# alexandervakhitov/lld-slam

Hardware: AMD Instinct MI355X
Metric: local-BA windows/sec (50 KF, 10k pts, 2k lines) at matched chi2; 1/2/4/8 GPU (higher is better)
Workload: dtype f64

## Files before the change

### lld_slam_amd/csrc/lld_ba.hip

```cpp
#include <algorithm>
#include <atomic>
#include <cfloat>
#include <chrono>
#include <cmath>
#include <cstdio>
#include <cstdlib>
#include <cstring>
#include <memory>
#include <mutex>
#include <new>
#include <thread>

#include "lld_ba_kernels.h"

using namespace lldba;

namespace {
constexpr int kNumPhases = 5;
constexpr int kFusePairsBelowWindows = 24;
constexpr int kMaxSuperSteps = 512;
constexpr int kChunkSmall = 4, kChunkFromWindows = 24;
constexpr int kSchurWindowTile = 8;
#ifdef LLD_EXPERIMENTS
static int exp_int(const char* name, int dflt) { const char* e = std::getenv(name); return e ? std::atoi(e) : dflt; }
// ... 431 lines not shown
    }
  if (!cholplan::build(n_free, adj, force, S.plan)) std::memset(&S.plan, 0, sizeof S.plan);
}

}


static void ba_drop_groups(lld_ba_batch* B) {
  for (auto& G : B->groups) {
    if (G.own_stream && G.st) (void)hipStreamSynchronize(G.st);
    if (G.gexec) { (void)hipGraphExecDestroy(G.gexec); G.gexec = nullptr; }
    if (G.graph) { (void)hipGraphDestroy(G.graph); G.graph = nullptr; }
    if (B->borrowed) continue;
    for (auto& row : G.ev) for (auto& e : row) if (e) (void)hipEventDestroy(e);
    if (G.own_stream && G.st) (void)hipStreamDestroy(G.st);
  }
  B->groups.clear();
}

static int ba_make_groups(lld_ba_batch* B, int n_groups) {
  const int n_windows = B->n_windows;
  int G = n_groups;
  if (G <= 0) {
    G = n_windows >= 16 ? 4 : (n_windows >= 8 ? 3 : 1);
    if (B->pipelined) G = std::min(G, 2);
    static const int groups_exp = exp_int("LLD_BA_GROUPS", 0);
    if (groups_exp >= 1 && groups_exp <= 8) G = groups_exp;
  }
  G = std::max(1, std::min(std::min(G, 8), n_windows));
  ba_drop_groups(B);
  B->groups.resize(G);
  for (int g = 0; g < G; g++) {
    lld_ba_batch::Group& Gr = B->groups[g];
    Gr.w0 = (int)((long long)n_windows * g / G); Gr.nw = (int)((long long)n_windows * (g + 1) / G) - Gr.w0;
    lld_ctx::BACache& cache = B->ctx->ba;
    if (g == 0) Gr.st = B->ctx->stream;
    else if (B->borrowed) {
      if (!cache.streams[g - 1]) LLD_HIP_TRY(hipStreamCreateWithFlags(&cache.streams[g - 1], hipStreamNonBlocking));
      Gr.st = cache.streams[g - 1]; Gr.own_stream = true;
    } else { LLD_HIP_TRY(hipStreamCreateWithFlags(&Gr.st, hipStreamNonBlocking)); Gr.own_stream = true; }
    Gr.d_counters = B->d_counters + 4 * g; Gr.h_counters = B->h_counters + 4 * g;
    static const int chunk_from = exp_int("LLD_BA_CHUNK_FROM", kChunkFromWindows);
    Gr.chunk0 = (B->pcg_multi || Gr.nw >= chunk_from) ? 1 : kChunkSmall; Gr.chunk = Gr.chunk0;
    Gr.chunk_from = chunk_from;
    for (int q = 0; q < Gr.chunk; q++)
      for (int k = 0; k < kNumPhases + 1; k++) {
        if (B->borrowed) { if (!cache.events[g][q][k]) LLD_HIP_TRY(hipEventCreate(&cache.events[g][q][k])); Gr.ev[q][k] = cache.events[g][q][k]; }
        else LLD_HIP_TRY(hipEventCreate(&Gr.ev[q][k]));
      }
    for (int wi = Gr.w0; wi < Gr.w0 + Gr.nw; wi++) {
      const BAWin& W = B->h_wins[wi];
      Gr.max_lblocks = std::max(Gr.max_lblocks, W.nb_pt + W.nb_ln);
      Gr.max_nt_pt = std::max(Gr.max_nt_pt, W.nt_pt); Gr.max_nb_ln = std::max(Gr.max_nb_ln, W.nt_ln);
      Gr.max_nl_pt = std::max(Gr.max_nl_pt, W.nl_pt); Gr.max_nl_ln = std::max(Gr.max_nl_ln, W.nl_ln);
      Gr.max_items_pt = std::max(Gr.max_items_pt, W.n_items_pt); Gr.max_items_ln = std::max(Gr.max_items_ln, W.n_items - W.n_items_pt);
      Gr.max_blk = std::max(Gr.max_blk, B->A.s_skip_empty ? W.n_blk_nz : W.n_free * (W.n_free + 1) / 2);
      const bool sp = (size_t)wi < B->plan_mode.size() && B->plan_mode[wi] == 1;
      Gr.any_sparse = Gr.any_sparse || sp; Gr.any_dense = Gr.any_dense || !sp;
    }
  }
  return LLD_OK;
}

extern "C" {

constexpr int kNotPacked = -1000;
static int ba_batch_create_impl(lld_ctx* ctx, int n_windows, const lld_ba_window* wins, const lld_ba_params* params, bool packed, lld_ba_batch** out) {
  if (!ctx || n_windows <= 0 || !wins || !out) return LLD_ERR_INVALID;
  *out = nullptr;
  for (int w = 0; w < n_windows; w++) { int st = validate_window(wins[w], false); if (st) return st; }
  LLD_HIP_TRY(hipSetDevice(ctx->device));
  static const bool timing = exp_flag("LLD_BA_TIMING");
  const auto tc0 = std::chrono::steady_clock::now();
  auto lap = [&](const char* what) { if (timing) std::fprintf(stderr, "[ba_create] %s at %.3f ms\n", what, std::chrono::duration<double, std::milli>(std::chrono::steady_clock::now() - tc0).count()); };
  lld_ba_batch* B = new lld_ba_batch();
  B->ctx = ctx; B->n_windows = n_windows;
  if (params) B->params = *params; else lld_ba_params_default(&B->params);
  const lld_ba_params& P = B->params;
  if (P.its_round1 < 1 || (P.protocol == 0 && P.its_round2 < 1) || P.its_round2 < 0 || P.max_trials <= 0 || !(P.pcg_rel_tol > 0) || P.reduced_solver < 0 || P.reduced_solver > 5 || P.protocol < 0 || P.protocol > 1 || P.abort_after_trials < 0) { delete B; return LLD_ERR_INVALID; }

  B->h_wins.resize(n_windows);
  B->chunk_landmarks = n_windows >= 64 ? 256 : (n_windows >= 8 ? 64 : 32);
  { static const int chunk_exp = exp_int("LLD_BA_CHUNK", 0); if (chunk_exp >= 1 && chunk_exp <= 4096) B->chunk_landmarks = chunk_exp; }
  std::vector<WinBases> bases(n_windows + 1);
  {
    WinBases b{};
    for (int wi = 0; wi < n_windows; wi++) {
      bases[wi] = b;
      const lld_ba_window& w = wins[wi];
      b.NC += w.n_cams; b.NP += w.n_points; b.NL += w.n_lines; b.NPE += w.n_pt_obs; b.NLO += w.n_ln_obs; b.NF += w.n_free_cams;
      const size_t n = 6 * (size_t)w.n_free_cams;
      b.S_total += n * n; b.x_total += n;
    }
    bases[n_windows] = b;
  }
  const long long NC = bases[n_windows].NC, NP = bases[n_windows].NP, NL = bases[n_windows].NL, NPE = bases[n_windows].NPE, NLO = bases[n_windows].NLO, NF = bases[n_windows].NF;
  if (NPE > 0x3fffffffll || NLO > 0x1fffffffll || NC * 7 > 0x7fffffffll) { delete B; return LLD_ERR_UNSUPPORTED; }
  const size_t S_total = bases[n_windows].S_total, x_total = bases[n_windows].x_total;
  const size_t NLE = 2 * (size_t)NLO;
  lld_ctx::BACache& cache = ctx->ba;
  const bool cached = !cache.busy.exchange(true);
  void* priv_stage[2] = {nullptr, nullptr};
  bool uploads_queued = false;
  auto fail = [&](int st) {
    if (uploads_queued) {
      (void)hipStreamSynchronize(ctx->stream);
      if (B->borrowed) cache.stage_pending = false;
    }
    for (void* q : priv_stage) if (q) (void)hipHostFree(q);
    ba_drop_groups(B);
    if (B->borrowed) cache.busy = false;
    else {
      if (B->h_counters) (void)hipHostFree(B->h_counters);
      if (B->slab) (void)hipFree(B->slab);
    }
    delete B; return st;
  };
  if (cached) B->borrowed = true;
  SecA hA{}, dA{};
  lld_slab dryA; dryA.base = reinterpret_cast<char*>(256);
  carve_a(dryA, packed, NC, NP, NL, NPE, NLE, hA);
  const size_t bytesA = dryA.used;
  void* arenaA = nullptr;
  { const int gs = stage_arena(ctx, cached, 0, bytesA, &arenaA); if (gs) return fail(gs); if (!cached) priv_stage[0] = arenaA; }
  { lld_slab sl; sl.base = static_cast<char*>(arenaA); sl.size = bytesA; carve_a(sl, packed, NC, NP, NL, NPE, NLE, hA); }
  HostArrays H;
  H.packed = packed;
  H.cam_qt0.view(hA.cam_qt0, 7 * (size_t)NC); H.pt0.view(hA.pt0, 3 * (size_t)NP); H.ln_x0.view(hA.ln_x0, 3 * (size_t)NL); H.ln_dir.view(hA.ln_dir, 3 * (size_t)NL);
  H.ln_info.view(hA.ln_info, 256);
  H.pt_obs_start.view(hA.pt_obs_start, (size_t)NP + 1); H.ln_obs_start.view(hA.ln_obs_start, (size_t)NL + 1);
  H.pe_pt.view(hA.pe_pt, NPE);
  if (packed) {
    H.pe_obs.view(hA.pe_obs, NPE); H.pe_cs.view(hA.pe_cs, NPE); H.lo_seg.view(hA.lo_seg, NLE); H.lo_cs.view(hA.lo_cs, NLO); H.lo_ln.view(hA.lo_ln, NLO); H.lo_oct.view(hA.lo_oct, NLO);
  } else {
    H.pe_cam.view(hA.pe_cam, NPE); H.pe_u.view(hA.pe_u, NPE); H.pe_v.view(hA.pe_v, NPE); H.pe_ur.view(hA.pe_ur, NPE); H.pe_s.view(hA.pe_s, NPE);
    H.le_cam.view(hA.le_cam, NLE); H.le_ln.view(hA.le_ln, NLE); H.le_xs.view(hA.le_xs, NLE); H.le_ys.view(hA.le_ys, NLE); H.le_xe.view(hA.le_xe, NLE); H.le_ye.view(hA.le_ye, NLE);
    H.le_s.view(hA.le_s, NLE);
  }
  H.pt_obs_start.p[NP] = (int)NPE; H.ln_obs_start.p[NL] = (int)NLO;
  for (int i = 0; i < 255; i++) H.ln_info.p[i] = P.protocol == 1 ? 1.0 : lld::line_info(P.gamma, i);
  H.ln_info.p[255] = 0.0;
  bool big_map = false;
  for (int wi = 0; wi < n_windows; wi++) {
    const size_t nf = (size_t)wins[wi].n_free_cams, nc = (size_t)wins[wi].n_cams;
    if (nf > (size_t)kMaxFreeCamsLds || (nf * 27 + 8 + nc * 7) * sizeof(double) > 158 * 1024 || (8 + nc * 14 + nf * 6) * sizeof(double) > 158 * 1024) big_map = true;
    B->max_free = std::max(B->max_free, wins[wi].n_free_cams); B->max_cams = std::max(B->max_cams, wins[wi].n_cams);
  }
  const bool force_big = exp_flag("LLD_BA_FORCE_BIG");
  if (force_big) big_map = true;
  B->big = big_map;
  if (P.deterministic < 0 || P.deterministic > 2) return fail(LLD_ERR_INVALID);
  if (B->big && P.deterministic == 1) return fail(LLD_ERR_UNSUPPORTED);
  const bool det = P.deterministic != 0 && !B->big;
  auto lin_lds_bytes = [&](int copies) { return ((size_t)B->max_free * 27 * copies + 8 + (size_t)B->max_cams * 7) * sizeof(double); };
  int copies = B->big ? 1 : kAccCopies;
  while (!B->big && copies > 1 && lin_lds_bytes(copies) > 150 * 1024) copies >>= 1;
  if (!B->big && lin_lds_bytes(copies) > 158 * 1024) return fail(LLD_ERR_UNSUPPORTED);
  B->acc_copies[0] = B->acc_copies[1] = copies;
  B->lin_waves[0] = det ? copies : kLinThreads / 64;
  B->lin_waves[1] = det ? copies : (n_windows >= 64 ? 4 : kLinThreads / 64);
  if (const char* e = exp_str("LLD_BA_LIN_WAVES")) {
    int a = 0, c = 0;
    if (std::sscanf(e, "%d,%d", &a, &c) == 2 && a >= 1 && a <= 8 && c >= 1 && c <= 8) {
      B->lin_waves[0] = a; B->lin_waves[1] = c;
      if (det) { B->acc_copies[0] = a; B->acc_copies[1] = c; if (lin_lds_bytes(std::max(a, c)) > 158 * 1024) return fail(LLD_ERR_UNSUPPORTED); }
    }
  }
  std::vector<WinStage> stages(n_windows);
  int n_threads = 1;
  const bool staged_under_solve = g_big_solves_running[ctx->device & 63].load(std::memory_order_relaxed) > 0;
  if (n_windows >= 4) {
    n_threads = (int)std::min<unsigned>(std::max(1u, std::thread::hardware_concurrency()), 16u);
    if (g_big_solves_running[ctx->device & 63].load(std::memory_order_relaxed) > 0) n_threads = std::min(n_threads, staging_cap());
    if (const char* e = std::getenv("LLD_HOST_THREADS")) { const int v = std::atoi(e); if (v >= 1 && v <= 64) n_threads = v; }
    if (g_big_solves_running[ctx->device & 63].load(std::memory_order_relaxed) > 0) n_threads = std::min(n_threads, staging_cap());
    n_threads = std::min(n_threads, n_windows);
  }
  std::atomic<int> first_error{LLD_OK};
  auto for_windows = [&](auto&& body) {
    std::atomic<int> next{0};
    auto worker = [&]() {
      for (;;) {
        const int wi = next.fetch_add(1);
        if (wi >= n_windows || first_error.load() != LLD_OK) break;
        try { body(wi); } catch (...) { int ok = LLD_OK; first_error.compare_exchange_strong(ok, LLD_ERR_ALLOC); }
      }
    };
    std::vector<std::thread> pool;
    try { for (int t = 1; t < n_threads; t++) pool.emplace_back(worker); } catch (...) {}
    worker();
    for (auto& t : pool) t.join();
  };
  void* const early_slab = (cached && n_windows >= 32 && cache.slab && cache.slab_bytes >= bytesA + 4096 && !exp_flag("LLD_BA_POISON") && !exp_flag("LLD_BA_NO_EARLY_UPLOAD")) ? cache.slab : nullptr;
  const int n_ranges = early_slab ? std::min(8, n_windows / 16) : 0;
  std::unique_ptr<std::atomic<int>[]> range_left(n_ranges ? new std::atomic<int>[(size_t)n_ranges] : nullptr);
  auto range_lo = [&](int r) { return (int)((long long)n_windows * r / std::max(1, n_ranges)); };
  for (int r = 0; r < n_ranges; r++) range_left[(size_t)r].store(range_lo(r + 1) - range_lo(r));
  auto copy_rows = [&](const void* hbase, size_t elt, long long lo, long long hi) -> bool {
    if (!hbase || hi <= lo) return true;
    const char* h = static_cast<const char*>(hbase) + elt * (size_t)lo;
    char* d = static_cast<char*>(early_slab) + (h - static_cast<const char*>(arenaA));
    return hipMemcpyAsync(d, h, elt * (size_t)(hi - lo), hipMemcpyHostToDevice, ctx->stream) == hipSuccess;
  };
  auto early_copy = [&](int r) {
    if (hipSetDevice(ctx->device) != hipSuccess) { int ok = LLD_OK; first_error.compare_exchange_strong(ok, LLD_ERR_HIP); return; }
    const WinBases& a = bases[(size_t)range_lo(r)]; const WinBases& b = bases[(size_t)range_lo(r + 1)];
    bool ok = copy_rows(hA.cam_qt0, 7 * sizeof(double), a.NC, b.NC) && copy_rows(hA.pt0, 3 * sizeof(double), a.NP, b.NP) &&
              copy_rows(hA.ln_x0, 3 * sizeof(double), a.NL, b.NL) && copy_rows(hA.ln_dir, 3 * sizeof(double), a.NL, b.NL) &&
              copy_rows(hA.pt_obs_start, sizeof(int), a.NP, b.NP) && copy_rows(hA.ln_obs_start, sizeof(int), a.NL, b.NL) && copy_rows(hA.pe_pt, sizeof(int), a.NPE, b.NPE);
    if (packed)
      ok = ok && copy_rows(hA.pe_obs, sizeof(float4), a.NPE, b.NPE) && copy_rows(hA.pe_cs, sizeof(int), a.NPE, b.NPE) && copy_rows(hA.lo_seg, sizeof(float4), 2 * a.NLO, 2 * b.NLO) &&
           copy_rows(hA.lo_cs, sizeof(int), a.NLO, b.NLO) && copy_rows(hA.lo_ln, sizeof(int), a.NLO, b.NLO) && copy_rows(hA.lo_oct, sizeof(unsigned short), a.NLO, b.NLO);
    else
      ok = ok && copy_rows(hA.pe_cam, sizeof(int), a.NPE, b.NPE) && copy_rows(hA.pe_u, sizeof(double), a.NPE, b.NPE) && copy_rows(hA.pe_v, sizeof(double), a.NPE, b.NPE) &&
           copy_rows(hA.pe_ur, sizeof(double), a.NPE, b.NPE) && copy_rows(hA.pe_s, sizeof(double), a.NPE, b.NPE) &&
           copy_rows(hA.le_cam, sizeof(int), 2 * a.NLO, 2 * b.NLO) && copy_rows(hA.le_ln, sizeof(int), 2 * a.NLO, 2 * b.NLO) &&
           copy_rows(hA.le_xs, sizeof(double), 2 * a.NLO, 2 * b.NLO) && copy_rows(hA.le_ys, sizeof(double), 2 * a.NLO, 2 * b.NLO) && copy_rows(hA.le_xe, sizeof(double), 2 * a.NLO, 2 * b.NLO) &&
           copy_rows(hA.le_ye, sizeof(double), 2 * a.NLO, 2 * b.NLO) && copy_rows(hA.le_s, sizeof(double), 2 * a.NLO, 2 * b.NLO);
    if (!ok) { int e_ = LLD_OK; first_error.compare_exchange_strong(e_, LLD_ERR_HIP); }
  };
  auto window_staged = [&](int wi) {
    if (!n_ranges) return;
    int r = (int)(((long long)wi * n_ranges) / n_windows);
    while (r + 1 < n_ranges && wi >= range_lo(r + 1)) r++;
    while (r > 0 && wi < range_lo(r)) r--;
    if (range_left[(size_t)r].fetch_sub(1) == 1) early_copy(r);
  };
  if (n_ranges) uploads_queued = true;
  const auto lap1 = [&](const char* what) { if (n_windows == 1) lap(what); };
  for_windows([&](int wi) {
    const int st = validate_window(wins[wi]);
    if (st) { int ok = LLD_OK; first_error.compare_exchange_strong(ok, st); return; }
    BAWin& W = B->h_wins[wi];
    WinStage& S = stages[wi];
    stage_tasks(wins[wi], P, bases[wi], n_windows, B->lin_waves, det, W, S);
    lap1("tasks built");
    if (n_windows == 1 && wins[wi].n_pt_obs + wins[wi].n_ln_obs > 20000) {
      std::thread helper;
      bool helped = false;
      try { helper = std::thread([&]() { try { stage_chunks(wins[wi], 3, bases[wi], B->chunk_landmarks, S.cs[0]); } catch (...) { int ok = LLD_OK; first_error.compare_exchange_strong(ok, LLD_ERR_ALLOC); } }); helped = true; } catch (...) {}
      if (!stage_edges(wins[wi], P, bases[wi], W, S, H)) { int ok = LLD_OK; first_error.compare_exchange_strong(ok, kNotPacked); }
      lap1("edges flattened");
      stage_chunks(wins[wi], 4, bases[wi], B->chunk_landmarks, S.cs[1]);
      if (helped) helper.join(); else stage_chunks(wins[wi], 3, bases[wi], B->chunk_landmarks, S.cs[0]);
    } else {
      if (!stage_edges(wins[wi], P, bases[wi], W, S, H)) { int ok = LLD_OK; first_error.compare_exchange_strong(ok, kNotPacked); return; }
      lap1("edges flattened");
      window_staged(wi);
      stage_chunks(wins[wi], 3, bases[wi], B->chunk_landmarks, S.cs[0]);
      stage_chunks(wins[wi], 4, bases[wi], B->chunk_landmarks, S.cs[1]);
    }
    stage_csr(wins[wi].n_free_cams, S);
    W.n_blk_nz = S.n_blk_nz;
    {
      static const int plan_force = exp_int("LLD_BA_CHOL_FORCE", 0);
      stage_chol_plan(wins[wi].n_free_cams, P.reduced_solver == 0 ? plan_force : (P.reduced_solver == 4 ? 1 : (P.reduced_solver == 5 ? 2 : 3)), S);
    }
    lap1("chunks built");
  });
  if (first_error.load() != LLD_OK) return fail(first_error.load());
  struct Place { size_t ptask, ltask, chunk, lm, tab, cams, blk_start, blk_src, cam_start, cam_src, part, cpart; };
  std::vector<Place> place(n_windows + 1);
  size_t n_hpart = 0; long long NPART = 0; int max_blk = 0;
  {
    Place q{};
    for (int wi = 0; wi < n_windows; wi++) {
      place[wi] = q;
      const WinStage& S = stages[wi];
      BAWin& W = B->h_wins[wi];
      W.ptask_off = (int)q.ptask; W.ltask_off = (int)q.ltask; W.item_off = (int)q.chunk;
      W.n_items_pt = (int)S.cs[0].chunks.size(); W.n_items = W.n_items_pt + (int)S.cs[1].chunks.size();
      W.blk_csr_off = (int)q.blk_start; W.cam_csr_off = (int)q.cam_start;
      W.hpart_off = (long long)n_hpart; n_hpart += (size_t)(big_map ? 1 : W.nl_pt + W.nl_ln) * W.n_free * 27;
      W.part_off = (int)NPART; NPART += W.nt_pt + W.nt_ln;
      q.ptask += S.ptasks.size(); q.ltask += S.ltasks.size(); q.chunk += (size_t)W.n_items;
      q.lm += S.cs[0].sg_lm.size() + S.cs[1].sg_lm.size(); q.tab += S.cs[0].sg_tab.size() + S.cs[1].sg_tab.size(); q.cams += S.cs[0].sg_cams.size() + S.cs[1].sg_cams.size();
      q.blk_start += S.blk_start.size(); q.blk_src += S.blk_src.size(); q.cam_start += S.cam_start.size(); q.cam_src += S.cam_src.size();
      q.part += S.cs[0].n_part + S.cs[1].n_part; q.cpart += S.cs[0].n_cpart + S.cs[1].n_cpart;
      if (q.part * 4 > 0x7fffffffull || q.tab > 0x7fffffffull) return fail(LLD_ERR_UNSUPPORTED);
      for (int d = 0; d < 2; d++) B->schur_lds[d] = std::max(B->schur_lds[d], S.cs[d].lds_need);
      for (int d = 0; d < 2; d++) B->schur_wide_lds = std::max(B->schur_wide_lds, S.cs[d].wide_lds_need);
      if (B->schur_wide_lds > 64 * 1024) return fail(LLD_ERR_UNSUPPORTED);
      max_blk = std::max(max_blk, W.n_free * (W.n_free + 1) / 2);
      B->max_items_pt = std::max(B->max_items_pt, W.n_items_pt); B->max_items_ln = std::max(B->max_items_ln, W.n_items - W.n_items_pt);
      B->max_lblocks = std::max(B->max_lblocks, W.nb_pt + W.nb_ln);
      B->max_free = std::max(B->max_free, W.n_free);
      B->max_cams = std::max(B->max_cams, W.n_cams);
      B->rec_stride = std::max(B->rec_stride, record_bytes(W));
    }
    place[n_windows] = q;
  }
  const Place& tot = place[n_windows];
  const size_t n_part = tot.part, n_cpart = tot.cpart;
  B->pcg_multi = n_windows <= 8 && B->max_free * 6 > kCholMN && P.reduced_solver != 2;
  const bool s_skip_empty = (P.reduced_solver == 0 || P.reduced_solver >= 3) && B->max_free * 6 <= kCholMN && !B->pcg_multi;
  if (B->max_free > kMaxFreeCamsOneWg && !B->pcg_multi) return fail(LLD_ERR_UNSUPPORTED);
  if (B->max_cams > kPcgThreads && !B->pcg_multi) return fail(LLD_ERR_UNSUPPORTED);
  for (int wi = 0; wi < n_windows; wi++) { B->h_wins[wi].acc_copies[0] = B->acc_copies[0]; B->h_wins[wi].acc_copies[1] = B->acc_copies[1]; B->h_wins[wi].win_index = wi; B->h_wins[wi].big = B->big ? 1 : 0; }
  B->max_blk = max_blk;
  for (int wi = 0; wi < n_windows; wi++) B->h_wins[wi].rec_off = (long long)(B->rec_stride * (size_t)wi);
  const size_t rec_total = B->rec_stride * (size_t)n_windows;
  B->S_total = S_total; B->x_total = x_total;
  const SecBSizes zB{tot.blk_start, tot.blk_src, tot.cam_start, tot.cam_src, tot.lm, tot.tab, tot.cams, tot.chunk, tot.ptask, tot.ltask, n_windows};
  hipStream_t st = ctx->stream;
  BAArrays& A = B->A;
  SecB dB{};
  size_t offA = 0, offB = 0, bytesB = 0;
  auto carve = [&](lld_slab& sl) {
    std::memset(&A, 0, sizeof A);
    offA = sl.used; carve_a(sl, packed, NC, NP, NL, NPE, NLE, dA);
    offB = sl.used; carve_b(sl, zB, dB); bytesB = sl.used - offB;
    A.cam_qt0 = dA.cam_qt0; A.pt0 = dA.pt0; A.ln_x0 = dA.ln_x0; A.ln_dir = dA.ln_dir; A.pt_obs_start = dA.pt_obs_start; A.ln_obs_start = dA.ln_obs_start;
    A.pe_pt = dA.pe_pt; A.ln_info = dA.ln_info; A.packed = packed ? 1 : 0;
    A.pe_obs = dA.pe_obs; A.pe_cs = dA.pe_cs; A.lo_seg = dA.lo_seg; A.lo_cs = dA.lo_cs; A.lo_ln = dA.lo_ln; A.lo_oct = dA.lo_oct;
    A.pe_cam = dA.pe_cam; A.pe_u = dA.pe_u; A.pe_v = dA.pe_v; A.pe_ur = dA.pe_ur; A.pe_s = dA.pe_s;
    A.le_cam = dA.le_cam; A.le_ln = dA.le_ln; A.le_xs = dA.le_xs; A.le_ys = dA.le_ys; A.le_xe = dA.le_xe; A.le_ye = dA.le_ye; A.le_s = dA.le_s;
    A.blk_start = dB.blk_start; A.blk_perm = dB.blk_perm; A.blk_src = dB.blk_src; A.cam_start = dB.cam_start; A.cam_src = dB.cam_src;
    A.sg_lm = dB.sg_lm; A.sg_tab = dB.sg_tab; A.sg_cams = dB.sg_cams; A.sg_chunks = dB.chunks; A.ptasks = dB.ptasks; A.ltasks = dB.ltasks;
    B->d_wins = dB.wins; A.chol_plan = dB.plans;
    B->d_state = sl.take<BAState>(n_windows);
    A.NC = NC; A.NP = NP; A.NL = NL;
    A.cam_qt = sl.take<double>(2 * NC * 7 + 1);
    A.ptx = sl.take<double>(2 * NP + 1); A.pty = sl.take<double>(2 * NP + 1); A.ptz = sl.take<double>(2 * NP + 1);
    A.lqx = sl.take<double>(2 * NL + 1); A.lqy = sl.take<double>(2 * NL + 1); A.lqz = sl.take<double>(2 * NL + 1); A.lqw = sl.take<double>(2 * NL + 1); A.lal = sl.take<double>(2 * NL + 1);
    A.pe_flags = sl.take<uint8_t>(NPE + 1); A.le_flags = sl.take<uint8_t>(NLE + 1);
    A.pe_chi2 = sl.take<double>(NPE + 1); A.le_chi2 = sl.take<double>(NLE + 1);
    A.pe_ws = sl.take<double>((size_t)NPE + 1); A.lo_W = sl.take<double>((size_t)NLO * 24 + 1);
    A.pt_active = sl.take<uint8_t>(NP + 1); A.ln_active = sl.take<uint8_t>(NL + 1); A.ln_removed = sl.take<uint8_t>(NL + 1);
    A.pt_V = sl.take<double>((size_t)NP * 9 + 1); A.ln_V = sl.take<double>((size_t)NL * 14 + 1);
    A.hpp_part = sl.take<double>(n_hpart + 2);
    A.Hpp = sl.take<double>((size_t)NF * 21 + 1); A.bp = sl.take<double>((size_t)NF * 6 + 1);
    A.S = sl.take<double>(S_total + 1); A.bschur = sl.take<double>(x_total + 1); A.xp = sl.take<double>(x_total + 1);
    A.x_total = (long long)x_total; A.s_skip_empty = s_skip_empty ? 1 : 0;
    if (B->pcg_multi) { A.pcg_vec = sl.take<double>(4 * x_total + 4); A.pcg_mi = sl.take<double>((size_t)NF * 36 + 1); A.pcg_sc = sl.take<double>(8 * (size_t)n_windows + 8); }
    A.chi_part = sl.take<double>(NPART + 1); A.chi_part2 = sl.take<double>(NPART + 1); A.scale_part = sl.take<double>(NPART + 1);
    A.sp_part = sl.take<double>(n_part * 36 + 2); A.sp_cpart = sl.take<double>(n_cpart * 6 + 2);
    A.records = sl.take<unsigned char>(rec_total + 256);
#ifdef LLD_EXPERIMENTS
    A.chol_stamps = exp_flag("LLD_BA_CHOL_STAMPS") ? sl.take<long long>((size_t)n_windows * kCholStampWaves * kCholStampSlots) : nullptr;
#endif
    B->d_counters = sl.take<int>(4 * 8);
    B->d_slot_map = sl.take<int>(2 * ((size_t)n_windows + 1)); B->d_active_pub = sl.take<int>((size_t)n_windows + 1);
  };
  lap("host staging done");
  lld_slab dry; dry.base = reinterpret_cast<char*>(256);
  carve(dry);
  const size_t bytes = dry.used + 4096;
  bool slab_regrown = false;
  if (cached) {
    if (bytes > cache.slab_bytes) {
      slab_regrown = true;
      void* old_slab = cache.slab;
      cache.slab = nullptr; cache.slab_bytes = 0;
      if (old_slab && hipFree(old_slab) != hipSuccess) return fail(LLD_ERR_HIP);
      const size_t want = bytes + (bytes >> 4);
      if (hipMalloc(&cache.slab, want) != hipSuccess) return fail(LLD_ERR_ALLOC);
      cache.slab_bytes = want;
    }
    B->slab = cache.slab;
  } else if (hipMalloc(&B->slab, bytes) != hipSuccess) return fail(LLD_ERR_ALLOC);
  B->slab_bytes = bytes;
  lap("slab ready");
  const bool poison = exp_flag("LLD_BA_POISON");
  if (poison && hipMemsetAsync(B->slab, 0xFF, bytes, st) != hipSuccess) return fail(LLD_ERR_HIP);
  lld_slab sl; sl.base = (char*)B->slab; sl.size = bytes;
  carve(sl);
#ifdef LLD_EXPERIMENTS
  if (A.chol_stamps && hipMemsetAsync(A.chol_stamps, 0, sizeof(long long) * (size_t)n_windows * kCholStampWaves * kCholStampSlots, st) != hipSuccess) return fail(LLD_ERR_HIP);
#endif
  if (s_skip_empty && S_total > 0 && hipMemsetAsync(A.S, 0, S_total * sizeof(double), st) != hipSuccess) return fail(LLD_ERR_HIP);
  uploads_queued = true;
  if (n_ranges && !slab_regrown && B->slab == early_slab && offA == 0) {
    bool ok = copy_rows(hA.ln_info, sizeof(double), 0, 256) && copy_rows(hA.pt_obs_start, sizeof(int), NP, NP + 1) && copy_rows(hA.ln_obs_start, sizeof(int), NL, NL + 1);
    if (!ok) return fail(LLD_ERR_HIP);
  } else if (hipMemcpyAsync((char*)B->slab + offA, arenaA, bytesA, hipMemcpyHostToDevice, st) != hipSuccess) return fail(LLD_ERR_HIP);
  lap("inputs queued");
  void* arenaB = nullptr;
  { const int gs = stage_arena(ctx, cached, 1, bytesB, &arenaB); if (gs) return fail(gs); if (!cached) priv_stage[1] = arenaB; }
  SecB hB{};
  B->plan_mode.assign((size_t)n_windows, 0);
  { lld_slab slb; slb.base = static_cast<char*>(arenaB); slb.size = bytesB; carve_b(slb, zB, hB); }
  hB.blk_start[tot.blk_start] = (int)tot.blk_src; hB.cam_start[tot.cam_start] = (int)tot.cam_src;
  for_windows([&](int wi) {
    const Place& q = place[wi];
    WinStage& S = stages[wi];
    std::copy(S.ptasks.begin(), S.ptasks.end(), hB.ptasks + q.ptask);
    std::copy(S.ltasks.begin(), S.ltasks.end(), hB.ltasks + q.ltask);
    size_t at_chunk = q.chunk, at_lm = q.lm, at_tab = q.tab, at_cams = q.cams;
    for (int d = 0; d < 2; d++) {
      const ChunkStage& C = S.cs[d];
      for (SChunk c : C.chunks) {
        c.lm_off += (int)at_lm; c.tab_off += (int)at_tab; c.cams_off += (int)at_cams; c.part_off += (int)q.part; c.cpart_off += (int)q.cpart;
        hB.chunks[at_chunk++] = c;
      }
      std::copy(C.sg_lm.begin(), C.sg_lm.end(), hB.sg_lm + at_lm); at_lm += C.sg_lm.size();
      std::copy(C.sg_tab.begin(), C.sg_tab.end(), hB.sg_tab + at_tab); at_tab += C.sg_tab.size();
      std::copy(C.sg_cams.begin(), C.sg_cams.end(), hB.sg_cams + at_cams); at_cams += C.sg_cams.size();
    }
    const int part4 = (int)(q.part * 4), cpart0 = (int)q.cpart, bsrc0 = (int)q.blk_src, csrc0 = (int)q.cam_src;
    for (size_t i = 0; i < S.blk_start.size(); i++) hB.blk_start[q.blk_start + i] = S.blk_start[i] + bsrc0;
    for (size_t i = 0; i < S.blk_perm.size(); i++) hB.blk_perm[q.blk_start + i] = S.blk_perm[i];
    for (size_t i = 0; i < S.blk_src.size(); i++) hB.blk_src[q.blk_src + i] = S.blk_src[i] + part4;
    for (size_t i = 0; i < S.cam_start.size(); i++) hB.cam_start[q.cam_start + i] = S.cam_start[i] + csrc0;
    for (size_t i = 0; i < S.cam_src.size(); i++) hB.cam_src[q.cam_src + i] = S.cam_src[i] + cpart0;
    hB.wins[wi] = B->h_wins[wi];
    hB.plans[wi] = S.plan; B->plan_mode[wi] = S.plan.mode;
    S = WinStage();
  });
  if (first_error.load() != LLD_OK) return fail(first_error.load());
  stages.clear();
  if (hipMemcpyAsync((char*)B->slab + offB, arenaB, bytesB, hipMemcpyHostToDevice, st) != hipSuccess) return fail(LLD_ERR_HIP);
  lap("structures queued");
  if (!cache.attrs_set || !cached) {
    const int lds_max = 159 * 1024;
    const void* fns[] = {reinterpret_cast<const void*>(ba_pcg_kernel), reinterpret_cast<const void*>(ba_backsub_pt_kernel), reinterpret_cast<const void*>(ba_backsub_ln_kernel),
                         reinterpret_cast<const void*>(ba_backsub_ctl_kernel), reinterpret_cast<const void*>(ba_linearize_pt_kernel), reinterpret_cast<const void*>(ba_linearize_ln_kernel),
                         reinterpret_cast<const void*>(ba_linearize_both_kernel), reinterpret_cast<const void*>(ba_backsub_pt_f64_kernel), reinterpret_cast<const void*>(ba_backsub_ln_f64_kernel),
                         reinterpret_cast<const void*>(ba_linearize_pt_f64_kernel), reinterpret_cast<const void*>(ba_linearize_ln_f64_kernel), reinterpret_cast<const void*>(ba_chol_kernel), reinterpret_cast<const void*>(ba_chol_mfma_kernel), reinterpret_cast<const void*>(ba_chol_sparse_kernel),
    };
    for (const void* f : fns) if (hipFuncSetAttribute(f, hipFuncAttributeMaxDynamicSharedMemorySize, lds_max) != hipSuccess) return fail(LLD_ERR_HIP);
    if (cached) cache.attrs_set = true;
  }
  lap("attributes set");
  if (B->borrowed) {
    if (!ctx->poll && hipHostMalloc(&ctx->poll, 256, hipHostMallocDefault) != hipSuccess) return fail(LLD_ERR_HIP);
    B->h_counters = static_cast<int*>(ctx->poll);
  } else if (hipHostMalloc((void**)&B->h_counters, 256, hipHostMallocDefault) != hipSuccess) return fail(LLD_ERR_HIP);
  B->h_abort = B->h_counters + 48;
  lap("pinned counters");
  B->pipelined = n_windows >= kSerialiseSolvesFromWindows && (staged_under_solve || g_big_solves_running[ctx->device & 63].load(std::memory_order_relaxed) > 0);
  { int gs = ba_make_groups(B, 0); if (gs) return fail(gs); }
  lap("groups made");
  if (cached) {
    if (!cache.stage_free && hipEventCreateWithFlags(&cache.stage_free, hipEventDisableTiming) != hipSuccess) return fail(LLD_ERR_HIP);
    if (hipEventRecord(cache.stage_free, st) != hipSuccess) return fail(LLD_ERR_HIP);
    cache.stage_pending = true;
  } else {
    if (hipStreamSynchronize(st) != hipSuccess) return fail(LLD_ERR_HIP);
    for (void*& q : priv_stage) if (q) { (void)hipHostFree(q); q = nullptr; }
  }
  lap("done");
  *out = B;
  return LLD_OK;
}

static int ba_batch_create_any(lld_ctx* ctx, int n_windows, const lld_ba_window* wins, const lld_ba_params* params, lld_ba_batch** out) {
  const bool f64_only = exp_flag("LLD_BA_OBS_F64");
  int st = f64_only ? kNotPacked : ba_batch_create_impl(ctx, n_windows, wins, params, true, out);
  if (st == kNotPacked) st = ba_batch_create_impl(ctx, n_windows, wins, params, false, out);
  return st;
}

int lld_ba_batch_create(lld_ctx* ctx, int n_windows, const lld_ba_window* wins, const lld_ba_params* params, lld_ba_batch** out) {
  return ba_batch_create_any(ctx, n_windows, wins, params, out);
}

struct StopFlag {
  volatile const int* i32; volatile const unsigned char* u8;
  bool up() const { return (i32 && *i32) || (u8 && *u8); }
};

static int ba_batch_solve_body(lld_ba_batch* B, StopFlag abort_flag, hipEvent_t t_begin, hipEvent_t t_end) {
  lld_ctx* ctx = B->ctx;
  std::unique_lock<std::mutex> turn(g_big_solve[ctx->device & 63], std::defer_lock);
  struct RunningGuard { std::atomic<int>* c; ~RunningGuard() { if (c) c->fetch_sub(1, std::memory_order_relaxed); } } running{nullptr};
  if (B->n_windows >= kSerialiseSolvesFromWindows) {
    turn.lock();
    running.c = &g_big_solves_running[ctx->device & 63]; running.c->fetch_add(1, std::memory_order_relaxed);
  }
  BAArrays& A = B->A;
  B->records_valid = false;
  for (auto& m : B->phase_ms) m = 0.0;
  for (auto& l : B->launches) l = 0;
  B->super_steps = 0;
  LLD_HIP_TRY(hipEventRecord(t_begin, ctx->stream));
  const size_t lin_lds_pt = B->big ? 64 : ((size_t)B->max_free * 27 * B->acc_copies[0] + 8 + (size_t)B->max_cams * 7) * sizeof(double);
  const size_t lin_lds_ln = B->big ? 64 : ((size_t)B->max_free * 27 * B->acc_copies[1] + 8 + (size_t)B->max_cams * 7) * sizeof(double);
  const bool same_lin_shape = B->lin_waves[0] == B->lin_waves[1] && B->acc_copies[0] == B->acc_copies[1];
  const size_t bs_lds = B->big ? 64 : (8 + (size_t)B->max_cams * 14 + (size_t)B->max_free * 6) * sizeof(double);
  const size_t pcg_lds = ((size_t)B->max_free * 6 * 4 + kPcgThreads + (size_t)B->max_free * 36 + 32) * sizeof(double);
  const size_t chol_fixed = ((size_t)B->max_free * 36 * 2 + (size_t)B->max_free * 6 * 2 + 32) * sizeof(double);
  const size_t chol_tri = std::min((size_t)B->max_free * (B->max_free + 1) / 2 * 36 * sizeof(double), (size_t)(156 * 1024) - chol_fixed) / 288 * 288;
  const size_t chol_lds = chol_fixed + chol_tri;
  const bool abort_at_start = abort_flag.up();
  *B->h_abort = 0;
  const bool live_flag = abort_flag.i32 != nullptr || abort_flag.u8 != nullptr;
  using Group = lld_ba_batch::Group;

  auto finalize_group = [&](Group& G) {
    const BAWin* dw = B->d_wins + G.w0; BAState* ds = B->d_state + G.w0;
    hipLaunchKernelGGL(ba_finalize_kernel, dim3(G.max_lblocks + 1, G.nw), dim3(kLmThreads), 0, G.st, A, dw, ds);
    hipLaunchKernelGGL(ba_mark_done_kernel, dim3((G.nw + 63) / 64), dim3(64), 0, G.st, ds, G.nw);
  };
  const bool use_slots = !(B->params.reduced_solver == 1 || B->pcg_multi);
  auto group_arrays = [&](const Group& G) { BAArrays Ag = B->A; int* rd = B->d_slot_map + (size_t)G.map_parity * ((size_t)B->n_windows + 1) + G.w0;
                                            int* wr = B->d_slot_map + (size_t)(G.map_parity ^ 1) * ((size_t)B->n_windows + 1) + G.w0;
                                            Ag.slot_map = use_slots ? wr : nullptr; Ag.active_pub = use_slots ? B->d_active_pub + G.w0 : nullptr;
                                            Ag.slot_rd = (use_slots && G.rows < G.nw) ? rd : nullptr; return Ag; };
  static const bool use_graph = exp_flag("LLD_BA_GRAPH");
  bool capturing = false;
  int n_superstep_launches = 0;
  const int fail_at = exp_int("LLD_BA_FAIL_AT_SUPERSTEP", -1);
  auto launch_superstep = [&](Group& G, int q) -> int {
    const BAWin* dw = B->d_wins + G.w0; BAState* ds = B->d_state + G.w0;
    if (fail_at >= 0 && n_superstep_launches++ == fail_at) return LLD_ERR_UNSUPPORTED;
    const BAArrays A = group_arrays(G);
    const int nw = use_slots ? std::max(1, std::min(G.rows, G.nw)) : G.nw; hipStream_t st = G.st;
    const int abort_now = abort_flag.up() ? 1 : 0;
    hipEvent_t* ev = G.ev[q];
    const bool tev = B->phase_events && !capturing;
    if (tev) LLD_HIP_TRY(hipEventRecord(ev[0], st));
    static const int fuse_below = exp_int("LLD_BA_FUSE_BELOW", kFusePairsBelowWindows);
    const bool packed = A.packed != 0;
    const bool fuse_pairs = nw < fuse_below && !B->big && packed;
    static const int fuse_bs_below = exp_int("LLD_BA_FUSE_BS_BELOW", -1);
    const bool fuse_bs = fuse_bs_below >= 0 ? (nw < fuse_bs_below && !B->big && packed) : fuse_pairs;
    if (B->big) {
      if (G.max_nl_pt > 0) hipLaunchKernelGGL(ba_linearize_pt_big_kernel, dim3(G.max_nl_pt, nw), dim3(64 * B->lin_waves[0]), lin_lds_pt, st, A, dw, ds);
      if (G.max_nl_ln > 0) hipLaunchKernelGGL(ba_linearize_ln_big_kernel, dim3(G.max_nl_ln, nw), dim3(64 * B->lin_waves[1]), lin_lds_ln, st, A, dw, ds);
    } else if (fuse_pairs && same_lin_shape && G.max_nl_pt > 0 && G.max_nl_ln > 0) hipLaunchKernelGGL(ba_linearize_both_kernel, dim3(G.max_nl_pt + G.max_nl_ln, nw), dim3(64 * B->lin_waves[0]), lin_lds_pt, st, A, dw, ds, G.max_nl_pt);
    else {
      if (G.max_nl_pt > 0) hipLaunchKernelGGL(packed ? ba_linearize_pt_kernel : ba_linearize_pt_f64_kernel, dim3(G.max_nl_pt, nw), dim3(64 * B->lin_waves[0]), lin_lds_pt, st, A, dw, ds);
      if (G.max_nl_ln > 0) hipLaunchKernelGGL(packed ? ba_linearize_ln_kernel : ba_linearize_ln_f64_kernel, dim3(G.max_nl_ln, nw), dim3(64 * B->lin_waves[1]), lin_lds_ln, st, A, dw, ds);
    }
    hipLaunchKernelGGL(ba_hpp_reduce_kernel, dim3(std::max(1, (B->max_free * 27 + 255) / 256), nw), dim3(256), 0, st, A, dw, ds);
    if (tev) LLD_HIP_TRY(hipEventRecord(ev[1], st));
    static const int schur_tile = std::max(1, exp_int("LLD_BA_SCHUR_TILE", kSchurWindowTile));
    static const bool split_schur = exp_flag("LLD_BA_SPLIT_SCHUR");
    if (split_schur) {
      if (G.max_items_pt > 0) hipLaunchKernelGGL(ba_schur_items_kernel<3>, dim3(G.max_items_pt, nw), dim3(kSchurThreads), B->schur_lds[0], st, A, dw, ds);
      if (G.max_items_ln > 0) hipLaunchKernelGGL(ba_schur_items_kernel<4>, dim3(G.max_items_ln, nw), dim3(kSchurThreads), B->schur_lds[1], st, A, dw, ds);
    } else if (G.max_items_pt + G.max_items_ln > 0) {
      if ((long long)nw * (G.max_items_pt + G.max_items_ln) * kSchurThreads > 0xffffffffll) return LLD_ERR_UNSUPPORTED;
      hipLaunchKernelGGL(ba_schur_items_both_kernel, dim3((unsigned)((long long)nw * (G.max_items_pt + G.max_items_ln))), dim3(kSchurThreads), std::max(B->schur_lds[0], B->schur_lds[1]), st, A, dw, ds, G.max_items_pt, schur_tile, nw, G.max_items_pt + G.max_items_ln);
    }
    if (B->schur_wide_lds > 0) hipLaunchKernelGGL(ba_schur_wide_kernel, dim3(G.max_items_pt + G.max_items_ln, nw), dim3(kSchurWideThreads), B->schur_wide_lds, st, A, dw, ds);
    hipLaunchKernelGGL(ba_schur_reduce_kernel, dim3((std::max(1, G.max_blk) * 6 + 255) / 256 + 2, nw), dim3(256), 0, st, A, dw, ds);
    if (B->params.reduced_solver == 1 || B->pcg_multi) hipLaunchKernelGGL(ba_symmetrize_kernel, dim3(B->pcg_multi ? 256 : 16, nw), dim3(256), 0, st, A, dw, ds);
    if (tev) LLD_HIP_TRY(hipEventRecord(ev[2], st));
    if (B->pcg_multi) {
      hipLaunchKernelGGL(ba_pcgm_init_kernel, dim3(nw), dim3(kPcgThreads), 0, st, A, dw, ds, B->params.pcg_rel_tol);
      const int n_max = B->max_free * 6, limit = B->params.pcg_max_iter > 0 ? B->params.pcg_max_iter : 10 * n_max;
      std::vector<double> hsc(8 * (size_t)nw);
      for (int it = 0; it < limit;) {
        for (int k = 0; k < 16 && it < limit; k++, it++) {
          hipLaunchKernelGGL(ba_pcgm_matvec_kernel, dim3((n_max + 3) / 4, nw), dim3(256), 0, st, A, dw);
          hipLaunchKernelGGL(ba_pcgm_update_kernel, dim3(nw), dim3(kPcgThreads), 0, st, A, dw, B->params.pcg_max_iter);
        }
        LLD_HIP_TRY(hipMemcpyAsync(hsc.data(), A.pcg_sc + 8 * (size_t)G.w0, hsc.size() * sizeof(double), hipMemcpyDeviceToHost, st));
        LLD_HIP_TRY(hipStreamSynchronize(st));
        bool all_done = true;
        for (int wI = 0; wI < nw; wI++) all_done = all_done && hsc[8 * (size_t)wI + 3] != 0.0;
        if (all_done) break;
      }
      hipLaunchKernelGGL(ba_pcgm_final_kernel, dim3(nw), dim3(kPcgThreads), 0, st, A, dw, ds);
    } else if (B->params.reduced_solver == 1)
      hipLaunchKernelGGL(ba_pcg_kernel, dim3(nw), dim3(kPcgThreads), pcg_lds, st, A, dw, ds, B->params.pcg_rel_tol, B->params.pcg_max_iter);
    else if ((B->params.reduced_solver == 0 || B->params.reduced_solver >= 3) && B->max_free * 6 <= kCholMN) {
      if (G.any_sparse) hipLaunchKernelGGL(ba_chol_sparse_kernel, dim3(nw), dim3(kSpThreads), kSpLdsBytes, st, A, dw, ds);
      if (G.any_dense) hipLaunchKernelGGL(ba_chol_mfma_kernel, dim3(nw), dim3(kCholMThreads), kCholMLdsDoubles * sizeof(double), st, A, dw, ds);
    }
    else
      hipLaunchKernelGGL(ba_chol_kernel, dim3(nw), dim3(kPcgThreads), chol_lds, st, A, dw, ds, (int)(chol_tri / sizeof(double)));
    if (tev) LLD_HIP_TRY(hipEventRecord(ev[3], st));
    bool control_fused = false;
    if (B->big) {
      if (G.max_nt_pt > 0) hipLaunchKernelGGL(ba_backsub_pt_big_kernel, dim3(G.max_nt_pt, nw), dim3(kLmThreads), bs_lds, st, A, dw, ds);
      if (G.max_nb_ln > 0) hipLaunchKernelGGL(ba_backsub_ln_big_kernel, dim3(G.max_nb_ln, nw), dim3(kLmThreads), bs_lds, st, A, dw, ds);
    } else if (fuse_bs && G.max_nt_pt > 0 && G.max_nb_ln > 0) {
      hipLaunchKernelGGL(ba_backsub_ctl_kernel, dim3(G.max_nt_pt + G.max_nb_ln, nw), dim3(kLmThreads), bs_lds, st, A, dw, ds, G.max_nt_pt, abort_now, G.nw, G.d_counters, G.h_counters,
                         (live_flag && G.chunk > 1) ? B->h_abort : nullptr);
      control_fused = true;
    }
    else {
      if (G.max_nt_pt > 0) hipLaunchKernelGGL(packed ? ba_backsub_pt_kernel : ba_backsub_pt_f64_kernel, dim3(G.max_nt_pt, nw), dim3(kLmThreads), bs_lds, st, A, dw, ds);
      if (G.max_nb_ln > 0) hipLaunchKernelGGL(packed ? ba_backsub_ln_kernel : ba_backsub_ln_f64_kernel, dim3(G.max_nb_ln, nw), dim3(kLmThreads), bs_lds, st, A, dw, ds);
    }
    if (tev) LLD_HIP_TRY(hipEventRecord(ev[4], st));
    if (!control_fused)
      hipLaunchKernelGGL(ba_control_kernel, dim3(nw), dim3(kCtlThreads), 0, st, A, dw, ds, abort_now, G.nw, G.d_counters, G.h_counters, (live_flag && G.chunk > 1) ? B->h_abort : nullptr);
    if (G.chunk > 1) {
      hipLaunchKernelGGL(ba_classify_kernel, dim3(std::max(1, G.max_lblocks), nw), dim3(kLmThreads), 0, st, A, dw, ds);
    }
    LLD_HIP_TRY(hipGetLastError());
    if (!capturing && (tev || q == G.chunk - 1)) LLD_HIP_TRY(hipEventRecord(ev[5], st));
    G.map_parity ^= 1;
    return LLD_OK;
  };
  auto launch_chunk = [&](Group& G) -> int {
    if (use_graph && G.chunk > 1 && (G.chunk & 1) == 0) {
      if (!G.gexec) {
        G.rows = G.nw;
        LLD_HIP_TRY(hipStreamBeginCapture(G.st, hipStreamCaptureModeThreadLocal));
        capturing = true;
        int s_ = LLD_OK;
        for (int q = 0; q < G.chunk && s_ == LLD_OK; q++) s_ = launch_superstep(G, q);
        capturing = false;
        LLD_HIP_TRY(hipStreamEndCapture(G.st, &G.graph));
        if (s_) return s_;
        LLD_HIP_TRY(hipGraphInstantiate(&G.gexec, G.graph, nullptr, nullptr, 0));
      }
      LLD_HIP_TRY(hipGraphLaunch(G.gexec, G.st));
      LLD_HIP_TRY(hipEventRecord(G.ev[G.chunk - 1][5], G.st));
      return LLD_OK;
    }
    for (int q = 0; q < G.chunk; q++) { const int s_ = launch_superstep(G, q); if (s_) return s_; }
    return LLD_OK;
  };

  for (Group& G : B->groups) {
    const BAWin* dw = B->d_wins + G.w0; BAState* ds = B->d_state + G.w0;
    if (G.own_stream) LLD_HIP_TRY(hipStreamWaitEvent(G.st, t_begin, 0));
    G.steps = 0; G.active = !abort_at_start; G.rows = G.nw; G.chunk = G.chunk0; G.map_parity = 0;
    LLD_HIP_TRY(hipMemsetAsync(G.d_counters, 0, 4 * sizeof(int), G.st));
    hipLaunchKernelGGL(ba_init_kernel, dim3(std::max(1, std::min(64, G.max_lblocks + 1)), G.nw), dim3(kLmThreads), 0, G.st, group_arrays(G), dw, ds);
    LLD_HIP_TRY(hipGetLastError());
    if (abort_at_start) {
      std::vector<BAState> hs(G.nw);
      std::memset(hs.data(), 0, sizeof(BAState) * G.nw);
      for (auto& s : hs) { s.phase = PH_FINALIZE; s.aborted = 1; }
      LLD_HIP_TRY(hipMemcpyAsync(ds, hs.data(), sizeof(BAState) * G.nw, hipMemcpyHostToDevice, G.st));
      LLD_HIP_TRY(hipStreamSynchronize(G.st));
      finalize_group(G);
    } else {
      int s = launch_chunk(G); if (s) return s;
    }
  }
  for (bool any = !abort_at_start; any;) {
    any = false;
    for (Group& G : B->groups) {
      if (!G.active) continue;
      if (live_flag && G.chunk > 1) {
        for (;;) {
          const hipError_t q = hipEventQuery(G.ev[G.chunk - 1][5]);
          if (q == hipSuccess) break;
          if (q != hipErrorNotReady) LLD_HIP_TRY(q);
          if (abort_flag.up()) __atomic_store_n(B->h_abort, 1, __ATOMIC_RELEASE);
          std::this_thread::yield();
        }
      } else LLD_HIP_TRY(hipEventSynchronize(G.ev[G.chunk - 1][5]));
      for (int q = 0; q < G.chunk; q++)
        for (int k = 0; k < kNumPhases; k++) {
          float ms = 0.f;
          if (B->phase_events && hipEventElapsedTime(&ms, G.ev[q][k], G.ev[q][k + 1]) == hipSuccess) B->phase_ms[k] += ms;
          B->launches[k]++;
        }
      G.steps += G.chunk; B->super_steps += G.chunk;
      const int n_run = G.h_counters[0], n_trans = G.h_counters[1], n_fin = G.h_counters[2];
      const BAWin* dw = B->d_wins + G.w0; BAState* ds = B->d_state + G.w0;
      if (use_slots && !(use_graph && G.gexec)) G.rows = n_run + n_trans;
      if (turn.owns_lock() && use_slots) {
        int left = 0;
        for (const Group& Gq : B->groups) left += Gq.active ? Gq.rows : 0;
        if (left * 8 <= B->n_windows) turn.unlock();
      }
      if (n_trans > 0 && G.chunk == 1) {
        hipLaunchKernelGGL(ba_classify_kernel, dim3(std::max(1, G.max_lblocks), use_slots ? std::max(1, G.rows) : G.nw), dim3(kLmThreads), 0, G.st, group_arrays(G), dw, ds);
      }
      (void)n_fin;
      LLD_HIP_TRY(hipGetLastError());
      if ((n_run + n_trans) > 0 && G.steps < kMaxSuperSteps) { int s = launch_chunk(G); if (s) return s; any = true; }
      else G.active = false;
    }
  }
  for (Group& G : B->groups) {
    finalize_group(G);
    LLD_HIP_TRY(hipGetLastError());
    if (G.own_stream) { LLD_HIP_TRY(hipEventRecord(G.ev[0][0], G.st)); LLD_HIP_TRY(hipStreamWaitEvent(ctx->stream, G.ev[0][0], 0)); }
  }
  LLD_HIP_TRY(hipEventRecord(t_end, ctx->stream));
  LLD_HIP_TRY(hipEventSynchronize(t_end));
  float tot = 0.f;
  (void)hipEventElapsedTime(&tot, t_begin, t_end);
// ... 238 lines not shown
```

### lld_slam_amd/csrc/lld_ba_kernels.h

```cpp
#ifndef LLD_BA_KERNELS_H
#define LLD_BA_KERNELS_H

#include "lld_common.h"
#include "lld_device_math.h"
#include "lld_ba_chol_plan.h"

namespace lldba {

using namespace lld;

constexpr int kLmThreads = 256;
constexpr int kSchurThreads = 64;
constexpr int kSchurWideThreads = 256;
constexpr int kPcgThreads = 1024;
constexpr int kCtlThreads = 64;
constexpr int kLinThreads = 512;
constexpr int kRoundsThroughput[4] = {8, 2, 4, 1};
constexpr int kRoundsLatency[4] = {4, 2, 4, 1};
constexpr int kRoundsThroughputMinWindows = 32;
constexpr int kRoundsThroughputBig[4] = {16, 4, 16, 1};
constexpr int kRoundsBigMinWindows = 192;
constexpr int kAccCopies = 4;
constexpr int kAccCopiesDoc = 4;
constexpr int kMaxFreeCams = 8192;
constexpr int kMaxFreeCamsLds = 590;
constexpr int kMaxFreeCamsOneWg = 170;

enum Phase : int { PH_RUN = 0, PH_TRANSITION = 2, PH_FINALIZE = 3, PH_DONE = 4 };
constexpr uint8_t EF_LEVEL1 = 1, EF_ROBUST = 2, EF_VALID = 4, EF_PAIRSTEREO = 8, EF_STEREO = 16;

struct BAWin {
  CamK cam;
  int n_cams, n_free;
  int cam_off;
  int pt_off, n_pt;
  int ln_off, n_ln;
  int pe_off, n_pe;
  int le_off, n_le;
  int hpp_off;
  int x_off;
  long long S_off;
  int item_off, n_items, n_items_pt;
  int lo_off, n_lo;
  int blk_csr_off, cam_csr_off;
  int n_blk_nz;
  int nb_pt, nb_ln;
  int ptask_off, n_ptasks, nt_pt;
  int ltask_off, n_ltasks, nt_ln;
  int nl_pt, nl_ln;
  int rounds[4];
  long long hpart_off;
  int part_off;
  int its[2];
  int max_trials, ln_filter;
  int abort_after;
  int big;
  int protocol, robust_pts;
  int acc_copies[2];
  int det, lin_waves[2];
  int win_index;
  double th_mono, th_stereo;
  double th_ln_mono, th_ln_stereo;
  long long rec_off;
};

struct BAState {
  int phase, need_lin, round, it, q, cur, nBad, pcg_ok;
  double lambda, ni, currentChi, iniChi, scale_cam;
  unsigned long long maxdiag_bits;
  double chi2_round1, chi2_final;
  int lm_iterations[2], lm_trials[2];
  int pcg_iterations, aborted, n_active_edges, pad;
  int ticket_lin, ticket_bs, ticket_cls, pad2;
};

struct PTask { int l0, nl, e0, ne, ms, pad0, pad1, pad2; };

struct SChunk { int lm_off, n_lm, tab_off, cams_off, k, D, part_off, cpart_off; };

struct BAArrays {
  long long NC, NP, NL;
  double* cam_qt;
  double *ptx, *pty, *ptz;
  double *lqx, *lqy, *lqz, *lqw, *lal;
  const double* cam_qt0;
  const double* pt0;
  const double *ln_x0, *ln_dir;
  const int* pt_obs_start;
  const int* ln_obs_start;
  const int* pe_pt;
  int packed;
  int* slot_map;
  int* active_pub;
  const int* slot_rd;
  const float4* pe_obs;
  const int* pe_cs;
  const float4* lo_seg;
  const int* lo_cs;
  const int* lo_ln;
  const unsigned short* lo_oct;
  const double* ln_info;
  const int* pe_cam;
  const double *pe_u, *pe_v, *pe_ur, *pe_s;
  const int* le_cam; const int* le_ln;
  const double *le_xs, *le_ys, *le_xe, *le_ye, *le_s;
  uint8_t *pe_flags, *le_flags;
  double *pe_chi2, *le_chi2;
  double *pe_ws;
  double *lo_W;
  uint8_t *pt_active, *ln_active, *ln_removed;
  double *pt_V;
  double *ln_V;
  double *hpp_part;
  double *Hpp;
  double *bp;
  double *S, *bschur, *xp;
  double *pcg_vec;
  double *pcg_mi;
  double *pcg_sc;
  long long x_total;
  double *chi_part, *chi_part2, *scale_part;
  const SChunk* sg_chunks;
  const PTask* ptasks; const PTask* ltasks;
  double *sp_part, *sp_cpart;
  const int *blk_start, *blk_src, *cam_start, *cam_src;
  int s_skip_empty;
  const int *blk_perm;
  const int *sg_lm, *sg_tab, *sg_cams;
  const CholPlan* chol_plan;
  unsigned char* records;
#ifdef LLD_EXPERIMENTS
  long long* chol_stamps;
#endif
};
constexpr int kCholStampSlots = 256;
constexpr int kCholStampWaves = 16;
#ifdef LLD_EXPERIMENTS
#define LLD_CHOL_STAMP(k) do { if (stamp_base && lane == 0) stamp_base[(k)] = (long long)__builtin_amdgcn_s_memtime(); } while (0)
#else
#define LLD_CHOL_STAMP(k) do { } while (0)
#endif

__device__ __forceinline__ void xwg_store(double* p, double v) { __hip_atomic_store(p, v, __ATOMIC_RELAXED, __HIP_MEMORY_SCOPE_AGENT); }
__device__ __forceinline__ double xwg_load(const double* p) { return __hip_atomic_load(p, __ATOMIC_RELAXED, __HIP_MEMORY_SCOPE_AGENT); }
__device__ __forceinline__ void xwg_stores_done() { asm volatile("s_waitcnt vmcnt(0)" ::: "memory"); }
__device__ __forceinline__ void xwg_store_i32(int* p, int v) { __hip_atomic_store(p, v, __ATOMIC_RELAXED, __HIP_MEMORY_SCOPE_AGENT); }
__device__ __forceinline__ int xwg_load_i32(const int* p) { return __hip_atomic_load(p, __ATOMIC_RELAXED, __HIP_MEMORY_SCOPE_AGENT); }
#define LLD_ROW_WINDOW(A, st, y) ((A).slot_rd ? (A).slot_rd[(y)] : (int)(y))
__device__ __forceinline__ double wave_sum(double x) {
#pragma unroll
  for (int off = 32; off > 0; off >>= 1) x += __shfl_xor(x, off);
  return x;
}
__device__ __forceinline__ double wave_max(double x) {
#pragma unroll
  for (int off = 32; off > 0; off >>= 1) x = fmax(x, __shfl_xor(x, off));
  return x;
}
__device__ __forceinline__ double block_sum(double x, double* scratch) {
  const int lane = threadIdx.x & 63, wave = threadIdx.x >> 6, nw = blockDim.x >> 6;
  x = wave_sum(x);
  __syncthreads();
  if (lane == 0) scratch[wave] = x;
  __syncthreads();
  double t = 0.0;
  for (int i = 0; i < nw; i++) t += scratch[i];
  return t;
}
__device__ __forceinline__ double block_max(double x, double* scratch) {
  const int lane = threadIdx.x & 63, wave = threadIdx.x >> 6, nw = blockDim.x >> 6;
  x = wave_max(x);
  __syncthreads();
  if (lane == 0) scratch[wave] = x;
  __syncthreads();
  double t = 0.0;
  for (int i = 0; i < nw; i++) t = fmax(t, scratch[i]);
  return t;
}

template <int D>
__device__ __forceinline__ bool spd_inverse(const double* A, double* Ainv) {
  double L[D][D];
  bool ok = true;
#pragma unroll
  for (int j = 0; j < D; j++) {
    double d = A[j * D + j];
#pragma unroll
    for (int k = 0; k < j; k++) d -= L[j][k] * L[j][k];
    if (!(d > 0.0)) ok = false;
    const double ljj = sqrt(d);
    L[j][j] = ljj;
    const double inv = 1.0 / ljj;
#pragma unroll
    for (int i = j + 1; i < D; i++) {
      double s = A[i * D + j];
#pragma unroll
      for (int k = 0; k < j; k++) s -= L[i][k] * L[j][k];
      L[i][j] = s * inv;
    }
  }
  double Li[D][D];
#pragma unroll
  for (int j = 0; j < D; j++) {
    Li[j][j] = 1.0 / L[j][j];
#pragma unroll
    for (int i = j + 1; i < D; i++) {
      double s = 0.0;
#pragma unroll
      for (int k = j; k < i; k++) s -= L[i][k] * Li[k][j];
      Li[i][j] = s / L[i][i];
    }
  }
#pragma unroll
  for (int i = 0; i < D; i++)
#pragma unroll
    for (int j = i; j < D; j++) {
      double s = 0.0;
#pragma unroll
      for (int k = j; k < D; k++) s += Li[k][i] * Li[k][j];
      Ainv[i * D + j] = s; Ainv[j * D + i] = s;
    }
  return ok;
}

template <int D>
__device__ __forceinline__ void chol_packed(const double* U, double lambda, double* L, double* idiag) {
  double F[D][D];
  int kk = 0;
#pragma unroll
  for (int i = 0; i < D; i++)
#pragma unroll
    for (int j = i; j < D; j++) { F[j][i] = U[kk++]; }
#pragma unroll
  for (int i = 0; i < D; i++) F[i][i] += lambda;
#pragma unroll
  for (int j = 0; j < D; j++) {
    double d = F[j][j];
#pragma unroll
    for (int m = 0; m < j; m++) d -= L[j * (j + 1) / 2 + m] * L[j * (j + 1) / 2 + m];
    const double inv = rsqrt_nr(d);
    idiag[j] = inv;
#pragma unroll
    for (int i = j + 1; i < D; i++) {
      double sacc = F[i][j];
#pragma unroll
      for (int m = 0; m < j; m++) sacc -= L[i * (i + 1) / 2 + m] * L[j * (j + 1) / 2 + m];
      L[i * (i + 1) / 2 + j] = sacc * inv;
    }
  }
}
template <int D>
__device__ __forceinline__ void chol_solve(const double* U, double lambda, const double* t, double* x) {
  double L[D * (D + 1) / 2], idg[D], y[D];
  chol_packed<D>(U, lambda, L, idg);
#pragma unroll
  for (int c = 0; c < D; c++) {
    double sacc = t[c];
#pragma unroll
    for (int m = 0; m < c; m++) sacc -= y[m] * L[c * (c + 1) / 2 + m];
    y[c] = sacc * idg[c];
  }
#pragma unroll
  for (int c = D - 1; c >= 0; c--) {
    double sacc = y[c];
#pragma unroll
    for (int m = c + 1; m < D; m++) sacc -= x[m] * L[m * (m + 1) / 2 + c];
    x[c] = sacc * idg[c];
// ... 128 lines not shown
```

### lld_slam_amd/csrc/lld_ba_lines.h

```cpp

struct LineGeom { Vec3 c0, c1, X1, X2; double alpha; };
__device__ __forceinline__ LineGeom line_geom(const LineQ& L) {
  const Mat3 Rl = line_rotation_t<true>(L);
  LineGeom G; G.c0 = mat_col(Rl, 0); G.c1 = mat_col(Rl, 1); G.alpha = L.alpha; G.X1 = L.alpha * G.c1; G.X2 = G.X1 + G.c0;
  return G;
}
struct LnObsIn { uint8_t fl[2]; double xs[2], ys[2], xe[2], ye[2], s[2]; };
template <int kPk>
__device__ __forceinline__ void line_obs_load(const BAArrays& A, int o, LnObsIn& I) {
#pragma unroll
  for (int side = 0; side < 2; side++) {
    const int e = 2 * o + side;
    I.fl[side] = A.le_flags[e];
    const LnSeg g = ln_seg_of<kPk>(A, e);
    I.xs[side] = g.xs; I.ys[side] = g.ys; I.xe[side] = g.xe; I.ye[side] = g.ye;
  }
  if (obs_packed<kPk>(A)) { const unsigned oc = A.lo_oct[o]; I.s[0] = A.ln_info[oc & 255u]; I.s[1] = A.ln_info[oc >> 8]; }
  else { I.s[0] = A.le_s[2 * o]; I.s[1] = A.le_s[2 * o + 1]; }
}
__device__ __forceinline__ double line_obs_linearize(const BAArrays& A, const BAWin& W, const Pose& T, int o, int c, const LineGeom& G, const LnObsIn& I,
                                                     double* hb, double* acc_lds) {
  const bool free_cam = c < W.n_free;
  double Wo[24], Jc0[12], r0[2] = {0.0, 0.0}, ws0 = 0.0;
#pragma unroll
  for (int i = 0; i < 24; i++) Wo[i] = 0.0;
#pragma unroll
  for (int i = 0; i < 12; i++) Jc0[i] = 0.0;
  double chi = 0.0;
  const Mat3 Rc = quat_rotation(T.q);
  const Vec3 X1m = pose_map(T, G.X1), X2m = pose_map(T, G.X2);
#pragma unroll
  for (int side = 0; side < 2; side++) {
    const int e = 2 * o + side;
    const uint8_t fl = I.fl[side];
    if (!(fl & EF_VALID) || (fl & EF_LEVEL1)) continue;
    double r[2]; LineAdj adj;
    line_residual_t<true>(W.cam, side == 1 ? W.cam.bx_right : 0.0, X1m, X2m, I.xs[side], I.ys[side], I.xe[side], I.ye[side], r, &adj);
    const double s = I.s[side];
    const double c2 = chi2_of(r, 2, s);
    A.le_chi2[e] = c2;
    double w = 1.0, rho0 = c2;
    if (fl & EF_ROBUST) rho0 = huber_nr(c2, (fl & EF_PAIRSTEREO) ? W.th_ln_stereo : W.th_ln_mono, &w);
    chi += rho0;
    const double ws = w * s;
    double Jc[12], Jl[8];
    line_jac_pose(adj, X1m, X2m, Jc);
    line_jac_line(adj, Rc, G.c0, G.c1, G.alpha, Jl);
    int k = 0;
#pragma unroll
    for (int a = 0; a < 4; a++) {
      hb[10 + a] -= ws * (Jl[a] * r[0] + Jl[4 + a] * r[1]);
#pragma unroll
      for (int d = a; d < 4; d++) hb[k++] += ws * (Jl[a] * Jl[d] + Jl[4 + a] * Jl[4 + d]);
    }
    if (free_cam) {
#pragma unroll
      for (int rr = 0; rr < 6; rr++)
#pragma unroll
        for (int a = 0; a < 4; a++) Wo[rr * 4 + a] += ws * (Jc[rr] * Jl[a] + Jc[6 + rr] * Jl[4 + a]);
      if (side == 0) {
#pragma unroll
        for (int i = 0; i < 12; i++) Jc0[i] = Jc[i];
        r0[0] = r[0]; r0[1] = r[1]; ws0 = ws;
      } else {
        double* ac = acc_lds + c * 27;
        int kk = 0;
#pragma unroll
        for (int rr = 0; rr < 6; rr++) {
          atomicAdd(&ac[21 + rr], -(ws0 * (Jc0[rr] * r0[0] + Jc0[6 + rr] * r0[1]) + ws * (Jc[rr] * r[0] + Jc[6 + rr] * r[1])));
#pragma unroll
          for (int cc = rr; cc < 6; cc++)
            atomicAdd(&ac[kk++], ws0 * (Jc0[rr] * Jc0[cc] + Jc0[6 + rr] * Jc0[6 + cc]) + ws * (Jc[rr] * Jc[cc] + Jc[6 + rr] * Jc[6 + cc]));
        }
        ws0 = 0.0;
      }
    }
  }
  if (free_cam) {
    double* Wb = A.lo_W + (size_t)o * 24;
#pragma unroll
    for (int i = 0; i < 24; i += 2) *reinterpret_cast<double2*>(Wb + i) = make_double2(Wo[i], Wo[i + 1]);
    if (ws0 != 0.0) {
      double* ac = acc_lds + c * 27;
      int kk = 0;
#pragma unroll
      for (int rr = 0; rr < 6; rr++) {
        atomicAdd(&ac[21 + rr], -ws0 * (Jc0[rr] * r0[0] + Jc0[6 + rr] * r0[1]));
#pragma unroll
        for (int cc = rr; cc < 6; cc++) atomicAdd(&ac[kk++], ws0 * (Jc0[rr] * Jc0[cc] + Jc0[6 + rr] * Jc0[6 + cc]));
      }
    }
  }
  return chi;
}

template <bool kBig, int kPk>
__device__ __forceinline__ void ba_linearize_ln_body(const BAArrays& A, const BAWin* __restrict__ wins, BAState* __restrict__ st, const int bx) {
  extern __shared__ __attribute__((aligned(16))) double lds[];
  const int wrow = LLD_ROW_WINDOW(A, st, blockIdx.y);
  if (wrow < 0) return;
  const BAWin W = wins[wrow];
  BAState& S = st[wrow];
  if (S.phase != PH_RUN || !S.need_lin) return;
  if ((int)bx >= W.nl_ln) return;
  const int nacc = W.n_free * 27;
  double* acc_all = kBig ? A.hpp_part + W.hpart_off : lds;
  const int copies = W.acc_copies[1];
  double* scratch = kBig ? lds : lds + copies * nacc;
  double* acc = acc_all;
  const int cur = S.cur;
  double* cams_l = scratch + 8;
  const double* cams = kBig ? A.cam_qt + ((size_t)cur * A.NC + W.cam_off) * 7 : cams_l;
  const int nthr = blockDim.x, nwv = W.lin_waves[1];
  if (!kBig) {
    for (int i = threadIdx.x; i < copies * nacc; i += nthr) acc_all[i] = 0.0;
    acc = acc_all + (W.det ? (int)(threadIdx.x >> 6) : (int)((threadIdx.x >> 3) & (copies - 1))) * nacc;
    for (int i = threadIdx.x; i < W.n_cams * 7; i += nthr) cams_l[i] = A.cam_qt[((size_t)cur * A.NC + W.cam_off) * 7 + i];
  }
  __syncthreads();
  const int lane = threadIdx.x & 63;
  double chi = 0.0, maxd = 0.0;
  for (int rnd = 0; rnd < W.rounds[1]; rnd++) {
    const int ti = (bx * W.rounds[1] + rnd) * nwv + __builtin_amdgcn_readfirstlane(threadIdx.x >> 6);
    if (ti >= W.n_ltasks) break;
    const PTask T = A.ltasks[W.ltask_off + ti];
    double hb[14];
#pragma unroll
    for (int i = 0; i < 14; i++) hb[i] = 0.0;
    if (T.nl > 1) {
      const bool has = lane < T.ne;
      const int o = T.e0 + (has ? lane : 0);
      int c, l_raw;
      ln_cam_lm_of<kPk>(A, o, T.l0, c, l_raw);
      LnObsIn I;
      line_obs_load<kPk>(A, o, I);
      const int l = has ? l_raw : -1 - lane;
      const int g = W.ln_off + (has ? l : T.l0);
      const LineQ Lq = load_ln(A, cur, g);
      const bool lm_act = has && A.ln_active[g];
      if (lm_act) chi += line_obs_linearize(A, W, pose_load(cams + c * 7), o, c, line_geom(Lq), I, hb, acc);
      seg_sum<14>(hb, l, lane, T.ms);
      if (lm_act && o == A.ln_obs_start[g]) {
        double* V = A.ln_V + (size_t)g * 14;
#pragma unroll
        for (int i = 0; i < 14; i++) V[i] = hb[i];
        maxd = fmax(maxd, fmax(fmax(fabs(hb[0]), fabs(hb[4])), fmax(fabs(hb[7]), fabs(hb[9]))));
      }
    } else {
      const int g = W.ln_off + T.l0;
      if (A.ln_active[g]) {
        const LineGeom G = line_geom(load_ln(A, cur, g));
        for (int sidx = lane; sidx < T.ne; sidx += 64) {
          const int o = T.e0 + sidx, c = ln_cam_of<kPk>(A, o);
          LnObsIn I;
          line_obs_load<kPk>(A, o, I);
          chi += line_obs_linearize(A, W, pose_load(cams + c * 7), o, c, G, I, hb, acc);
        }
        wave_sum_n<14>(hb);
        if (lane == 0) {
          double* V = A.ln_V + (size_t)g * 14;
#pragma unroll
          for (int i = 0; i < 14; i++) V[i] = hb[i];
          maxd = fmax(maxd, fmax(fmax(fabs(hb[0]), fabs(hb[4])), fmax(fabs(hb[7]), fabs(hb[9]))));
        }
      }
    }
  }
  const double chi_t = block_sum(chi, scratch);
  const double max_t = block_max(maxd, scratch);
  if (threadIdx.x == 0) {
    A.chi_part[W.part_off + W.nl_pt + bx] = chi_t;
    atomicMax(&S.maxdiag_bits, (unsigned long long)__double_as_longlong(max_t));
  }
  __syncthreads();
  if (kBig) return;
  double* dst = A.hpp_part + W.hpart_off + (size_t)(W.nl_pt + bx) * nacc;
  for (int i = threadIdx.x; i < nacc; i += nthr) {
    double v = 0.0;
    for (int q = 0; q < copies; q++) v += acc_all[q * nacc + i];
    dst[i] = v;
  }
}
__global__ __launch_bounds__(kLinThreads) void ba_linearize_ln_kernel(BAArrays A, const BAWin* __restrict__ wins, BAState* __restrict__ st) { ba_linearize_ln_body<false, 1>(A, wins, st, (int)blockIdx.x); }
__global__ __launch_bounds__(kLinThreads) void ba_linearize_ln_f64_kernel(BAArrays A, const BAWin* __restrict__ wins, BAState* __restrict__ st) { ba_linearize_ln_body<false, 0>(A, wins, st, (int)blockIdx.x); }
__global__ __launch_bounds__(kLinThreads) void ba_linearize_ln_big_kernel(BAArrays A, const BAWin* __restrict__ wins, BAState* __restrict__ st) { ba_linearize_ln_body<true, kPkRuntime>(A, wins, st, (int)blockIdx.x); }

__device__ __forceinline__ void line_obs_wtx(const BAArrays& A, const BAWin& W, int o, int c, const double* xp, double* t) {
  const double* Wb = A.lo_W + (size_t)o * 24;
#pragma unroll
  for (int k = 0; k < 4; k++) {
    double s = 0.0;
#pragma unroll
    for (int r = 0; r < 6; r++) s += Wb[r * 4 + k] * xp[c * 6 + r];
    t[k] = s;
  }
}
__device__ __forceinline__ double line_obs_trial(const BAArrays& A, const BAWin& W, const Pose& T, int o, const LineGeom& G, const LnObsIn& I) {
  double chi = 0.0;
  const Vec3 X1m = pose_map(T, G.X1), X2m = pose_map(T, G.X2);
#pragma unroll
  for (int side = 0; side < 2; side++) {
    const int e = 2 * o + side;
    const uint8_t fl = I.fl[side];
    if (!(fl & EF_VALID) || (fl & EF_LEVEL1)) continue;
    double r[2];
    line_residual_t<true>(W.cam, side == 1 ? W.cam.bx_right : 0.0, X1m, X2m, I.xs[side], I.ys[side], I.xe[side], I.ye[side], r, nullptr);
    const double c2 = chi2_of(r, 2, I.s[side]);
    A.le_chi2[e] = c2;
    double w, rho0 = c2;
    if (fl & EF_ROBUST) rho0 = huber_nr(c2, (fl & EF_PAIRSTEREO) ? W.th_ln_stereo : W.th_ln_mono, &w);
    chi += rho0;
  }
  return chi;
}
__device__ __forceinline__ double line_backsub(const double* V, double lambda, const double* wtx, const LineQ& L, LineQ& Ln) {
  double t[4], xl[4], sc = 0.0;
#pragma unroll
  for (int i = 0; i < 4; i++) t[i] = V[10 + i] - wtx[i];
  chol_solve<4>(V, lambda, t, xl);
#pragma unroll
  for (int i = 0; i < 4; i++) sc += xl[i] * (lambda * xl[i] + V[10 + i]);
  Ln = line_oplus(L, xl);
  return sc;
}

template <bool kBig, int kPk>
__device__ __forceinline__ void ba_backsub_ln_body(const BAArrays& A, const BAWin* __restrict__ wins, const BAState* __restrict__ st, const int bx) {
  extern __shared__ __attribute__((aligned(16))) double lds[];
  double* scratch = lds;
  const int wrow = LLD_ROW_WINDOW(A, st, blockIdx.y);
  if (wrow < 0) return;
  const BAWin W = wins[wrow];
  const BAState& S = st[wrow];
  if (S.phase != PH_RUN) return;
  if ((int)bx >= W.nt_ln) return;
  const int cur = S.cur, nxt = cur ^ 1;
  const double lambda = S.lambda;
  double* camB_l = lds + 8; double* xps_l = camB_l + W.n_cams * 7;
  const double* camB = kBig ? A.cam_qt + ((size_t)nxt * A.NC + W.cam_off) * 7 : camB_l;
  const double* xp = kBig ? A.xp + W.x_off : xps_l;
  const int task_wave = __builtin_amdgcn_readfirstlane(threadIdx.x >> 6);
  PTask T_next = A.ltasks[W.ltask_off + min((bx * W.rounds[3]) * 4 + task_wave, W.n_ltasks - 1)];
  if (!kBig) {
    for (int i = threadIdx.x; i < W.n_cams * 7; i += kLmThreads) camB_l[i] = A.cam_qt[((size_t)nxt * A.NC + W.cam_off) * 7 + i];
    for (int i = threadIdx.x; i < 6 * W.n_free; i += kLmThreads) xps_l[i] = A.xp[W.x_off + i];
  }
  __syncthreads();
  const int lane = threadIdx.x & 63;
  double chi = 0.0, sc = 0.0;
  for (int rnd = 0; rnd < W.rounds[3]; rnd++) {
    const int ti = (bx * W.rounds[3] + rnd) * 4 + task_wave;
    if (ti >= W.n_ltasks) break;
    const PTask T = T_next;
    T_next = A.ltasks[W.ltask_off + min((bx * W.rounds[3] + rnd + 1) * 4 + task_wave, W.n_ltasks - 1)];
    if (T.nl > 1) {
      const bool has = lane < T.ne;
      const int o = T.e0 + (has ? lane : 0);
      int c, l_raw;
      ln_cam_lm_of<kPk>(A, o, T.l0, c, l_raw);
      LnObsIn I;
      line_obs_load<kPk>(A, o, I);
      const bool lmk = lane < T.nl;
      const int g2 = W.ln_off + T.l0 + (lmk ? lane : 0);
      const LineQ L2 = load_ln(A, cur, g2);
      const int act2 = lmk ? (int)A.ln_active[g2] : 0;
      const int start2 = A.ln_obs_start[g2], end2 = A.ln_obs_start[g2 + 1];
      const int l = has ? l_raw : -1 - lane;
      const int slot = has ? l - T.l0 : 0;
      const bool lm_act = has && __shfl(act2, slot) != 0;
      double wtx[4] = {0, 0, 0, 0};
      if (lm_act && c < W.n_free) line_obs_wtx(A, W, o, c, xp, wtx);
      double V2[14];
#pragma unroll
      for (int i = 0; i < 14; i++) V2[i] = A.ln_V[(size_t)g2 * 14 + i];
      seg_sum<4>(wtx, l, lane, T.ms);
      const int first = (lmk && end2 > start2) ? start2 - T.e0 : 0;
      double wl[4];
#pragma unroll
      for (int i = 0; i < 4; i++) wl[i] = __shfl(wtx[i], first);
      LineQ Ln2 = L2;
      if (lmk) {
        if (act2 && end2 > start2) sc += line_backsub(V2, lambda, wl, L2, Ln2);
        store_ln(A, nxt, g2, Ln2);
      }
      LineQ Ln;
      Ln.q.x = __shfl(Ln2.q.x, slot); Ln.q.y = __shfl(Ln2.q.y, slot); Ln.q.z = __shfl(Ln2.q.z, slot); Ln.q.w = __shfl(Ln2.q.w, slot); Ln.alpha = __shfl(Ln2.alpha, slot);
      if (lm_act) chi += line_obs_trial(A, W, pose_load(camB + c * 7), o, line_geom(Ln), I);
    } else {
      const int g = W.ln_off + T.l0;
      const LineQ L = load_ln(A, cur, g);
      if (!A.ln_active[g]) { if (lane == 0) store_ln(A, nxt, g, L); }
      else {
        double wtx[4] = {0, 0, 0, 0};
        for (int sidx = lane; sidx < T.ne; sidx += 64) {
          const int o = T.e0 + sidx, c = ln_cam_of<kPk>(A, o);
          if (c >= W.n_free) continue;
          double t1[4];
          line_obs_wtx(A, W, o, c, xp, t1);
          wtx[0] += t1[0]; wtx[1] += t1[1]; wtx[2] += t1[2]; wtx[3] += t1[3];
        }
        wave_sum_n<4>(wtx);
        LineQ Ln;
        const double s1 = line_backsub(A.ln_V + (size_t)g * 14, lambda, wtx, L, Ln);
        if (lane == 0) { sc += s1; store_ln(A, nxt, g, Ln); }
        const LineGeom G = line_geom(Ln);
        for (int sidx = lane; sidx < T.ne; sidx += 64) {
          const int o = T.e0 + sidx;
          LnObsIn I;
          line_obs_load<kPk>(A, o, I);
          chi += line_obs_trial(A, W, pose_load(camB + ln_cam_of<kPk>(A, o) * 7), o, G, I);
        }
      }
    }
  }
  const double chi_t = block_sum(chi, scratch);
  const double sc_t = block_sum(sc, scratch);
  if (threadIdx.x == 0) { xwg_store(&A.chi_part2[W.part_off + W.nt_pt + bx], chi_t); xwg_store(&A.scale_part[W.part_off + W.nt_pt + bx], sc_t); xwg_stores_done(); }
}
__global__ __launch_bounds__(kLmThreads, 4) void ba_backsub_ln_kernel(BAArrays A, const BAWin* __restrict__ wins, const BAState* __restrict__ st) { ba_backsub_ln_body<false, 1>(A, wins, st, (int)blockIdx.x); }
__global__ __launch_bounds__(kLmThreads, 4) void ba_backsub_ln_f64_kernel(BAArrays A, const BAWin* __restrict__ wins, const BAState* __restrict__ st) { ba_backsub_ln_body<false, 0>(A, wins, st, (int)blockIdx.x); }
__global__ __launch_bounds__(kLmThreads) void ba_backsub_ln_big_kernel(BAArrays A, const BAWin* __restrict__ wins, const BAState* __restrict__ st) { ba_backsub_ln_body<true, kPkRuntime>(A, wins, st, (int)blockIdx.x); }

__global__ __launch_bounds__(kLinThreads) void ba_linearize_both_kernel(BAArrays A, const BAWin* __restrict__ wins, BAState* __restrict__ st, int n_pt_blocks) {
  if ((int)blockIdx.x < n_pt_blocks) ba_linearize_pt_body<false, 1>(A, wins, st, (int)blockIdx.x);
  else ba_linearize_ln_body<false, 1>(A, wins, st, (int)blockIdx.x - n_pt_blocks);
}

__device__ __forceinline__ void ba_begin_body(const BAArrays& A, const BAWin& W, BAState& S, int lane) {
  double chi = 0.0;
  const int nb = W.nl_pt + W.nl_ln;
  for (int i = lane; i < nb; i += 64) chi += A.chi_part[W.part_off + i];
  chi = wave_sum(chi);
  double md = 0.0;
  if (S.it == 0) {
    const double* H = A.Hpp + (size_t)W.hpp_off * 21;
    for (int c = lane; c < W.n_free; c += 64) {
      const double* h = H + c * 21;
      md = fmax(md, fmax(fmax(fabs(xwg_load(h)), fabs(xwg_load(h + 6))), fmax(fmax(fabs(xwg_load(h + 11)), fabs(xwg_load(h + 15))), fmax(fabs(xwg_load(h + 18)), fabs(xwg_load(h + 20))))));
    }
    md = wave_max(md);
  }
  if (lane == 0) {
    S.currentChi = chi; S.iniChi = chi;
    if (S.it == 0) {
      md = fmax(md, __longlong_as_double((long long)S.maxdiag_bits));
      S.lambda = 1e-5 * md; S.ni = 2.0; S.nBad = 0;
    }
    S.q = 0; S.need_lin = 0;
  }
}

__global__ __launch_bounds__(256) void ba_hpp_reduce_kernel(BAArrays A, const BAWin* __restrict__ wins, BAState* __restrict__ st) {
  __shared__ int is_last;
  const int wrow = LLD_ROW_WINDOW(A, st, blockIdx.y);
  if (wrow < 0) return;
  const BAWin W = wins[wrow];
  BAState& S = st[wrow];
  if (S.phase != PH_RUN || !S.need_lin) return;
  const int nacc = W.n_free * 27;
  const int i = blockIdx.x * 256 + threadIdx.x;
  if (i < nacc) {
    const double* src = A.hpp_part + W.hpart_off + i;
    const int nb = W.big ? 1 : W.nl_pt + W.nl_ln;
    double v = 0.0;
    int b = 0;
    for (; b + 8 <= nb; b += 8) {
      double t[8];
#pragma unroll
      for (int u = 0; u < 8; u++) t[u] = src[(size_t)(b + u) * nacc];
#pragma unroll
      for (int u = 0; u < 8; u++) v += t[u];
    }
    for (; b < nb; b++) v += src[(size_t)b * nacc];
    const int c = i / 27, k = i - c * 27;
    if (k < 21) xwg_store(&A.Hpp[((size_t)W.hpp_off + c) * 21 + k], v); else A.bp[((size_t)W.hpp_off + c) * 6 + (k - 21)] = v;
  }
  xwg_stores_done();
  __syncthreads();
  if (threadIdx.x == 0) is_last = atomicAdd(&S.ticket_lin, 1) == (int)gridDim.x - 1;
  __syncthreads();
  if (is_last && threadIdx.x < 64) {
    if (threadIdx.x == 0) S.ticket_lin = 0;
    ba_begin_body(A, W, S, threadIdx.x);
  }
}
```

### lld_slam_amd/csrc/lld_ba_points.h

```cpp

__device__ __forceinline__ int dpp_down1(int v) { return __builtin_amdgcn_mov_dpp(v, 0x130, 0xf, 0xf, true); }
__device__ __forceinline__ int dpp_up1(int v) { return __builtin_amdgcn_mov_dpp(v, 0x138, 0xf, 0xf, true); }
template <int OFF>
__device__ __forceinline__ int dpp_down(int v) {
#pragma unroll
  for (int h = 0; h < OFF; h++) v = dpp_down1(v);
  return v;
}
template <int OFF>
__device__ __forceinline__ double dpp_down(double v) {
  return __hiloint2double(dpp_down<OFF>(__double2hiint(v)), dpp_down<OFF>(__double2loint(v)));
}
__device__ __forceinline__ bool seg_step(int seg, int lane, int off) {
  const int so = __shfl_down(seg, off);
  return (lane + off < 64) && so == seg;
}
template <int N, int OFF>
__device__ __forceinline__ void seg_sum_step(double* v, int seg1) {
  const bool ok = dpp_down<OFF>(seg1) == seg1;
  double o[N];
#pragma unroll
  for (int i = 0; i < N; i++) o[i] = dpp_down<OFF>(v[i]);
  if (ok) {
#pragma unroll
    for (int i = 0; i < N; i++) v[i] += o[i];
  }
}
template <int N>
__device__ __forceinline__ void seg_sum(double* v, int seg, int lane, int max_len) {
  if (max_len > 1) seg_sum_step<N, 1>(v, seg + 1);
  if (max_len > 2) seg_sum_step<N, 2>(v, seg + 1);
  if (max_len > 4) seg_sum_step<N, 4>(v, seg + 1);
  for (int off = 8; off < max_len; off <<= 1) {
    const bool ok = seg_step(seg, lane, off);
#pragma unroll
    for (int i = 0; i < N; i++) { const double o = __shfl_down(v[i], off); if (ok) v[i] += o; }
  }
}
template <int N>
__device__ __forceinline__ void wave_sum_n(double* v) {
#pragma unroll
  for (int i = 0; i < N; i++) v[i] = wave_sum(v[i]);
}

struct PtEdgeLin { double r[3], Jp[9], Jc[18], ws, rho0; bool stereo; };

template <int kPk>
__device__ __forceinline__ void point_edge_linearize(const BAArrays& A, const BAWin& W, int cur, int e, uint8_t fl, int c, const Vec3& X, PtEdgeLin& L) {
  const Pose T = load_cam(A, cur, W.cam_off + c);
  const Vec3 Xc = pose_map(T, X);
  const PtObs ob = pt_obs_of<kPk>(A, e);
  L.stereo = !(ob.ur < 0);
  point_residual_iz(W.cam, Xc, rcp_nr(Xc.z), ob.u, ob.v, ob.ur, L.stereo, true, L.r);
  const double s = ob.s;
  const double c2 = chi2_of(L.r, L.stereo ? 3 : 2, s);
  A.pe_chi2[e] = c2;
  double w = 1.0;
  L.rho0 = c2;
  if (fl & EF_ROBUST) L.rho0 = huber_nr(c2, L.stereo ? W.th_stereo : W.th_mono, &w);
  L.ws = w * s;
  A.pe_ws[e] = L.stereo ? -L.ws : L.ws;
  point_jac_point(W.cam, Xc, quat_rotation(T.q), L.stereo, L.Jp);
  point_jac_pose(W.cam, Xc, L.stereo, L.Jc);
}
__device__ __forceinline__ void point_edge_hll(const PtEdgeLin& L, double* hb) {
  int k = 0;
#pragma unroll
  for (int a = 0; a < 3; a++)
#pragma unroll
    for (int d = a; d < 3; d++) hb[k++] = L.ws * (L.Jp[a] * L.Jp[d] + L.Jp[3 + a] * L.Jp[3 + d] + L.Jp[6 + a] * L.Jp[6 + d]);
#pragma unroll
  for (int a = 0; a < 3; a++) hb[6 + a] = -L.ws * (L.Jp[a] * L.r[0] + L.Jp[3 + a] * L.r[1] + L.Jp[6 + a] * L.r[2]);
}
__device__ __forceinline__ void point_edge_hpp(const PtEdgeLin& L, double* ac) {
  int kk = 0;
#pragma unroll
  for (int rr = 0; rr < 6; rr++) {
    atomicAdd(&ac[21 + rr], -L.ws * (L.Jc[rr] * L.r[0] + L.Jc[6 + rr] * L.r[1] + L.Jc[12 + rr] * L.r[2]));
#pragma unroll
    for (int cc = rr; cc < 6; cc++) atomicAdd(&ac[kk++], L.ws * (L.Jc[rr] * L.Jc[cc] + L.Jc[6 + rr] * L.Jc[6 + cc] + L.Jc[12 + rr] * L.Jc[12 + cc]));
  }
}

__device__ __forceinline__ double point_edge_blocks_closed(const BAWin& W, const Pose& T, const Vec3& X, const PtObs& ob, uint8_t fl, double& ws_out,
                                                           double& rho0_out, double* hb, double* hp) {
  const CamK& k = W.cam;
  const Vec3 Xc = pose_map(T, X);
  const bool stereo = !(ob.ur < 0);
  double r[3];
  const double iz = rcp_nr(Xc.z), iz2 = iz * iz;
  point_residual_iz(k, Xc, iz, ob.u, ob.v, ob.ur, stereo, true, r);
  const double c2e = chi2_of(r, stereo ? 3 : 2, ob.s);
  double w = 1.0, rho0 = c2e;
  if (fl & EF_ROBUST) rho0 = huber_nr(c2e, stereo ? W.th_stereo : W.th_mono, &w);
  const double ws = w * ob.s;
  ws_out = ws; rho0_out = rho0;
  const Mat3 R = quat_rotation(T.q);
  const double a = k.fx * iz, b = k.fy * iz;
  const double c0 = -k.fx * Xc.x * iz2, c1 = -k.fy * Xc.y * iz2, c2 = c0 + k.bf * iz2;
  const double m00 = ws * (stereo ? 2.0 * a * a : a * a);
  const double m02 = ws * (stereo ? a * (c0 + c2) : a * c0);
  const double m11 = ws * (b * b), m12 = ws * (b * c1);
  const double m22 = ws * (stereo ? c0 * c0 + c1 * c1 + c2 * c2 : c0 * c0 + c1 * c1);
  const double wr0 = ws * r[0], wr1 = ws * r[1], wr2 = stereo ? ws * r[2] : 0.0;
  const double g0 = a * (wr0 + wr2), g1 = b * wr1, g2 = c0 * wr0 + c1 * wr1 + c2 * wr2;
  double G[3][3];
#pragma unroll
  for (int j = 0; j < 3; j++) {
    G[0][j] = m00 * R.m[0][j] + m02 * R.m[2][j];
    G[1][j] = m11 * R.m[1][j] + m12 * R.m[2][j];
    G[2][j] = m02 * R.m[0][j] + m12 * R.m[1][j] + m22 * R.m[2][j];
  }
  int kk = 0;
#pragma unroll
  for (int p = 0; p < 3; p++)
#pragma unroll
    for (int d = p; d < 3; d++) hb[kk++] = R.m[0][p] * G[0][d] + R.m[1][p] * G[1][d] + R.m[2][p] * G[2][d];
#pragma unroll
  for (int p = 0; p < 3; p++) hb[6 + p] = R.m[0][p] * g0 + R.m[1][p] * g1 + R.m[2][p] * g2;
  const double x = Xc.x, y = Xc.y, z = Xc.z;
  const double P[3][3] = {{y * m02 - z * 0.0, y * m12 - z * m11, y * m22 - z * m12},
                          {z * m00 - x * m02, z * 0.0 - x * m12, z * m02 - x * m22},
                          {x * 0.0 - y * m00, x * m11 - y * 0.0, x * m12 - y * m02}};
  const double Q[3][3] = {{y * P[0][2] - z * P[0][1], z * P[0][0] - x * P[0][2], x * P[0][1] - y * P[0][0]},
                          {y * P[1][2] - z * P[1][1], z * P[1][0] - x * P[1][2], x * P[1][1] - y * P[1][0]},
                          {y * P[2][2] - z * P[2][1], z * P[2][0] - x * P[2][2], x * P[2][1] - y * P[2][0]}};
  hp[0] = Q[0][0]; hp[1] = Q[0][1]; hp[2] = Q[0][2]; hp[3] = P[0][0]; hp[4] = P[0][1]; hp[5] = P[0][2];
  hp[6] = Q[1][1]; hp[7] = Q[1][2]; hp[8] = P[1][0]; hp[9] = P[1][1]; hp[10] = P[1][2];
  hp[11] = Q[2][2]; hp[12] = P[2][0]; hp[13] = P[2][1]; hp[14] = P[2][2];
  hp[15] = m00; hp[16] = 0.0; hp[17] = m02; hp[18] = m11; hp[19] = m12; hp[20] = m22;
  hp[21] = y * g2 - z * g1; hp[22] = z * g0 - x * g2; hp[23] = x * g1 - y * g0; hp[24] = g0; hp[25] = g1; hp[26] = g2;
  return c2e;
}

template <bool kBig, int kPk>
__device__ __forceinline__ void ba_linearize_pt_body(const BAArrays& A, const BAWin* __restrict__ wins, BAState* __restrict__ st, const int bx) {
  extern __shared__ __attribute__((aligned(16))) double lds[];
  const int wrow = LLD_ROW_WINDOW(A, st, blockIdx.y);
  if (wrow < 0) return;
  const BAWin W = wins[wrow];
  BAState& S = st[wrow];
  if (S.phase != PH_RUN || !S.need_lin) return;
  if ((int)bx >= W.nl_pt) return;
  const int nacc = W.n_free * 27;
  const int cur = S.cur;
  double* acc_all = kBig ? A.hpp_part + W.hpart_off : lds;
  const int copies = W.acc_copies[0];
  double* scratch = kBig ? lds : lds + copies * nacc;
  double* cams_l = scratch + 8;
  const double* cams = kBig ? A.cam_qt + ((size_t)cur * A.NC + W.cam_off) * 7 : cams_l;
  double* acc = acc_all;
  const int nthr = blockDim.x, nwv = W.lin_waves[0];
  const int task_wave = __builtin_amdgcn_readfirstlane(threadIdx.x >> 6);
  PTask T_next = A.ptasks[W.ptask_off + min((bx * W.rounds[0]) * nwv + task_wave, W.n_ptasks - 1)];
  if (!kBig) {
    for (int i = threadIdx.x; i < copies * nacc; i += nthr) acc_all[i] = 0.0;
    acc = acc_all + (W.det ? (int)(threadIdx.x >> 6) : (int)((threadIdx.x >> 3) & (copies - 1))) * nacc;
    for (int i = threadIdx.x; i < W.n_cams * 7; i += nthr) cams_l[i] = A.cam_qt[((size_t)cur * A.NC + W.cam_off) * 7 + i];
  }
  __syncthreads();
  const int lane = threadIdx.x & 63;
  double chi = 0.0, maxd = 0.0;
  for (int rnd = 0; rnd < W.rounds[0]; rnd++) {
    const int ti = (bx * W.rounds[0] + rnd) * nwv + task_wave;
    if (ti >= W.n_ptasks) break;
    const PTask T = T_next;
    T_next = A.ptasks[W.ptask_off + min((bx * W.rounds[0] + rnd + 1) * nwv + task_wave, W.n_ptasks - 1)];
    if (T.nl > 1) {
      const bool has = lane < T.ne;
      const int e = T.e0 + (has ? lane : 0);
      int c, l_raw;
      pt_cam_lm_of<kPk>(A, e, T.l0, c, l_raw);
      const int l = has ? l_raw : -1 - lane;
      const uint8_t fl = A.pe_flags[e];
      const PtObs ob = pt_obs_of<kPk>(A, e);
      const bool lmk = lane < T.nl;
      const int g2 = W.pt_off + T.l0 + (lmk ? lane : 0);
      const Vec3 X2 = load_pt(A, cur, g2);
      const int act2 = lmk ? (int)A.pt_active[g2] : 0;
      const int slot = has ? l - T.l0 : 0;
      Vec3 X; X.x = __shfl(X2.x, slot); X.y = __shfl(X2.y, slot); X.z = __shfl(X2.z, slot);
      const bool lm_act = has && __shfl(act2, slot) != 0;
      const bool head = lm_act && dpp_up1(l + 1) != l + 1;
      double hb[9];
#pragma unroll
      for (int i = 0; i < 9; i++) hb[i] = 0.0;
      if (has && (fl & EF_LEVEL1)) A.pe_ws[e] = 0.0;
      if (lm_act && !(fl & EF_LEVEL1)) {
        double hp[27], ws_e, rho0_e;
        A.pe_chi2[e] = point_edge_blocks_closed(W, pose_load(cams + c * 7), X, ob, fl, ws_e, rho0_e, hb, hp);
        A.pe_ws[e] = (fl & EF_STEREO) ? -ws_e : ws_e;
        chi += rho0_e;
        if (c < W.n_free) {
          double* ac = acc + c * 27;
#pragma unroll
          for (int i = 0; i < 27; i++) if (i != 16) atomicAdd(&ac[i], hp[i]);
        }
      }
      seg_sum<9>(hb, l, lane, T.ms);
      if (head) {
        double* V = A.pt_V + (size_t)(W.pt_off + l) * 9;
#pragma unroll
        for (int i = 0; i < 9; i++) V[i] = hb[i];
        maxd = fmax(maxd, fmax(fabs(hb[0]), fmax(fabs(hb[3]), fabs(hb[5]))));
      }
    } else {
      const int g = W.pt_off + T.l0;
      if (A.pt_active[g]) {
        const Vec3 X = load_pt(A, cur, g);
        double hb[9];
#pragma unroll
        for (int i = 0; i < 9; i++) hb[i] = 0.0;
        for (int sidx = lane; sidx < T.ne; sidx += 64) {
          const int e = T.e0 + sidx;
          const uint8_t fl = A.pe_flags[e];
          if (fl & EF_LEVEL1) { A.pe_ws[e] = 0.0; continue; }
          const int c = pt_cam_of<kPk>(A, e);
          PtEdgeLin L;
          point_edge_linearize<kPk>(A, W, cur, e, fl, c, X, L);
          chi += L.rho0;
          double h1[9];
          point_edge_hll(L, h1);
#pragma unroll
          for (int i = 0; i < 9; i++) hb[i] += h1[i];
          if (c < W.n_free) point_edge_hpp(L, acc + c * 27);
        }
        wave_sum_n<9>(hb);
        if (lane == 0) {
          double* V = A.pt_V + (size_t)g * 9;
#pragma unroll
          for (int i = 0; i < 9; i++) V[i] = hb[i];
          maxd = fmax(maxd, fmax(fabs(hb[0]), fmax(fabs(hb[3]), fabs(hb[5]))));
        }
      }
    }
  }
  const double chi_t = block_sum(chi, scratch);
  const double max_t = block_max(maxd, scratch);
  if (threadIdx.x == 0) {
    A.chi_part[W.part_off + bx] = chi_t;
    atomicMax(&S.maxdiag_bits, (unsigned long long)__double_as_longlong(max_t));
  }
  __syncthreads();
  if (kBig) return;
  double* dst = A.hpp_part + W.hpart_off + (size_t)(bx) * nacc;
  for (int i = threadIdx.x; i < nacc; i += nthr) {
    double v = 0.0;
    for (int q = 0; q < copies; q++) v += acc_all[q * nacc + i];
    dst[i] = v;
  }
}
__global__ __launch_bounds__(kLinThreads, 4) void ba_linearize_pt_kernel(BAArrays A, const BAWin* __restrict__ wins, BAState* __restrict__ st) { ba_linearize_pt_body<false, 1>(A, wins, st, (int)blockIdx.x); }
__global__ __launch_bounds__(kLinThreads, 4) void ba_linearize_pt_f64_kernel(BAArrays A, const BAWin* __restrict__ wins, BAState* __restrict__ st) { ba_linearize_pt_body<false, 0>(A, wins, st, (int)blockIdx.x); }
__global__ __launch_bounds__(kLinThreads, 4) void ba_linearize_pt_big_kernel(BAArrays A, const BAWin* __restrict__ wins, BAState* __restrict__ st) { ba_linearize_pt_body<true, kPkRuntime>(A, wins, st, (int)blockIdx.x); }

__device__ __forceinline__ void point_edge_wtx(const BAArrays& A, const BAWin& W, int cur, int e, uint8_t fl, int c, const Vec3& X, const double* xp, double* t) {
  const double ws = fabs(A.pe_ws[e]);
  const bool stereo = (fl & EF_STEREO) != 0;
  const Pose T = load_cam(A, cur, W.cam_off + c);
  const Vec3 Xc = pose_map(T, X);
  double Jp[9], Jc[18];
  point_jac_point(W.cam, Xc, quat_rotation(T.q), stereo, Jp);
  point_jac_pose(W.cam, Xc, stereo, Jc);
  double uu[3];
#pragma unroll
  for (int i = 0; i < 3; i++) {
    double s = 0.0;
#pragma unroll
    for (int r = 0; r < 6; r++) s += Jc[i * 6 + r] * xp[c * 6 + r];
    uu[i] = ws * s;
  }
#pragma unroll
  for (int k = 0; k < 3; k++) t[k] = Jp[k] * uu[0] + Jp[3 + k] * uu[1] + Jp[6 + k] * uu[2];
}
template <int kPk>
__device__ __forceinline__ double point_edge_trial(const BAArrays& A, const BAWin& W, int nxt, int e, uint8_t fl, int c, const Vec3& Xn) {
  const Pose T = load_cam(A, nxt, W.cam_off + c);
  const Vec3 Xc = pose_map(T, Xn);
  const PtObs ob = pt_obs_of<kPk>(A, e);
  const bool stereo = !(ob.ur < 0);
  double r[3];
  point_residual_iz(W.cam, Xc, rcp_nr(Xc.z), ob.u, ob.v, ob.ur, stereo, true, r);
  const double c2 = chi2_of(r, stereo ? 3 : 2, ob.s);
  A.pe_chi2[e] = c2;
  double w, rho0 = c2;
  if (fl & EF_ROBUST) rho0 = huber_nr(c2, stereo ? W.th_stereo : W.th_mono, &w);
  return rho0;
}
__device__ __forceinline__ double point_backsub(const double* V, double lambda, const double* wtx, const Vec3& X, Vec3& Xn) {
  const double t[3] = {V[6] - wtx[0], V[7] - wtx[1], V[8] - wtx[2]};
  double xl[3], sc = 0.0;
  chol_solve<3>(V, lambda, t, xl);
#pragma unroll
  for (int i = 0; i < 3; i++) sc += xl[i] * (lambda * xl[i] + V[6 + i]);
  Xn = vec3(X.x + xl[0], X.y + xl[1], X.z + xl[2]);
  return sc;
}

template <bool kBig, int kPk>
__device__ __forceinline__ void ba_backsub_pt_body(const BAArrays& A, const BAWin* __restrict__ wins, const BAState* __restrict__ st, const int bx) {
  extern __shared__ __attribute__((aligned(16))) double lds[];
  const int wrow = LLD_ROW_WINDOW(A, st, blockIdx.y);
  if (wrow < 0) return;
  const BAWin W = wins[wrow];
  const BAState& S = st[wrow];
  if (S.phase != PH_RUN) return;
  if ((int)bx >= W.nt_pt) return;
  const int cur = S.cur, nxt = cur ^ 1;
  const double lambda = S.lambda;
  const double* xp = A.xp + W.x_off;
  double* scratch = lds;
  double* camA_l = lds + 8;
  double* camB_l = camA_l + W.n_cams * 7;
  double* xps_l = camB_l + W.n_cams * 7;
  const double* camA = kBig ? A.cam_qt + ((size_t)cur * A.NC + W.cam_off) * 7 : camA_l;
  const double* camB = kBig ? A.cam_qt + ((size_t)nxt * A.NC + W.cam_off) * 7 : camB_l;
  const double* xps = kBig ? xp : xps_l;
  const int task_wave = __builtin_amdgcn_readfirstlane(threadIdx.x >> 6);
  PTask T_next = A.ptasks[W.ptask_off + min((bx * W.rounds[2]) * 4 + task_wave, W.n_ptasks - 1)];
  if (!kBig) {
    for (int i = threadIdx.x; i < W.n_cams * 7; i += kLmThreads) {
      camA_l[i] = A.cam_qt[((size_t)cur * A.NC + W.cam_off) * 7 + i];
      camB_l[i] = A.cam_qt[((size_t)nxt * A.NC + W.cam_off) * 7 + i];
    }
    for (int i = threadIdx.x; i < 6 * W.n_free; i += kLmThreads) xps_l[i] = xp[i];
  }
  __syncthreads();
  const int lane = threadIdx.x & 63;
  double chi = 0.0, sc = 0.0;
  for (int rnd = 0; rnd < W.rounds[2]; rnd++) {
    const int ti = (bx * W.rounds[2] + rnd) * 4 + task_wave;
    if (ti >= W.n_ptasks) break;
    const PTask T = T_next;
    T_next = A.ptasks[W.ptask_off + min((bx * W.rounds[2] + rnd + 1) * 4 + task_wave, W.n_ptasks - 1)];
    if (T.nl > 1) {
      const bool has = lane < T.ne;
      const int e = T.e0 + (has ? lane : 0);
      int c, l_raw;
      pt_cam_lm_of<kPk>(A, e, T.l0, c, l_raw);
      const int l = has ? l_raw : -1 - lane;
      const uint8_t fl = A.pe_flags[e];
      const double ws = fabs(A.pe_ws[e]);
      const PtObs ob = pt_obs_of<kPk>(A, e);
      const bool lmk = lane < T.nl;
      const int g2 = W.pt_off + T.l0 + (lmk ? lane : 0);
      const Vec3 X2 = load_pt(A, cur, g2);
      const int act2 = lmk ? (int)A.pt_active[g2] : 0;
      const int start2 = A.pt_obs_start[g2], end2 = A.pt_obs_start[g2 + 1];
      double V2[9];
#pragma unroll
      for (int i = 0; i < 9; i++) V2[i] = A.pt_V[(size_t)g2 * 9 + i];
      const int slot = has ? l - T.l0 : 0;
      Vec3 X; X.x = __shfl(X2.x, slot); X.y = __shfl(X2.y, slot); X.z = __shfl(X2.z, slot);
      const bool e_act = has && __shfl(act2, slot) != 0 && !(fl & EF_LEVEL1);
      double wtx[3] = {0, 0, 0};
      if (e_act && c < W.n_free) {
        const Pose Tc = pose_load(camA + c * 7);
        const Vec3 Xc = pose_map(Tc, X);
        const bool stereo = (fl & EF_STEREO) != 0;
        const Mat3 R = quat_rotation(Tc.q);
        const double* xc = xps + c * 6;
        const Vec3 v = cross(Xc, vec3(xc[0], xc[1], xc[2])) - vec3(xc[3], xc[4], xc[5]);
        const double iz = rcp_nr(Xc.z), iz2 = iz * iz;
        const double a = W.cam.fx * iz, b = W.cam.fy * iz;
        const double c0 = -W.cam.fx * Xc.x * iz2, c1 = -W.cam.fy * Xc.y * iz2, c2 = c0 + W.cam.bf * iz2;
        const double u0 = ws * (a * v.x + c0 * v.z), u1 = ws * (b * v.y + c1 * v.z), u2 = stereo ? ws * (a * v.x + c2 * v.z) : 0.0;
        const double h0 = a * (u0 + u2), h1 = b * u1, h2 = c0 * u0 + c1 * u1 + c2 * u2;
#pragma unroll
        for (int k = 0; k < 3; k++) wtx[k] = -(R.m[0][k] * h0 + R.m[1][k] * h1 + R.m[2][k] * h2);
      }
      seg_sum<3>(wtx, l, lane, T.ms);
      const int first = (lmk && end2 > start2) ? start2 - T.e0 : 0;
      double wl[3];
#pragma unroll
      for (int i = 0; i < 3; i++) wl[i] = __shfl(wtx[i], first);
      Vec3 Xn2 = X2;
      if (lmk) {
        if (act2 && end2 > start2) sc += point_backsub(V2, lambda, wl, X2, Xn2);
        store_pt(A, nxt, g2, Xn2);
      }
      Vec3 Xn; Xn.x = __shfl(Xn2.x, slot); Xn.y = __shfl(Xn2.y, slot); Xn.z = __shfl(Xn2.z, slot);
      if (e_act) {
        const Vec3 Xc = pose_map(pose_load(camB + c * 7), Xn);
        const bool stereo = !(ob.ur < 0);
        double r[3];
        point_residual_iz(W.cam, Xc, rcp_nr(Xc.z), ob.u, ob.v, ob.ur, stereo, true, r);
        const double c2 = chi2_of(r, stereo ? 3 : 2, ob.s);
        A.pe_chi2[e] = c2;
        double w, rho0 = c2;
        if (fl & EF_ROBUST) rho0 = huber_nr(c2, stereo ? W.th_stereo : W.th_mono, &w);
        chi += rho0;
      }
    } else {
      const int g = W.pt_off + T.l0;
      const Vec3 X = load_pt(A, cur, g);
      if (!A.pt_active[g]) { if (lane == 0) store_pt(A, nxt, g, X); }
      else {
        double wtx[3] = {0, 0, 0};
// ... 31 lines not shown
```

### lld_slam_amd/csrc/lld_ba_schur.h

```cpp

constexpr int kSchurWideK = 64;

__host__ __device__ inline int schur_nb(int k) {
  int NB = 64 / k; if (NB < 1) NB = 1;
  const int np = k * (k + 1) / 2, units = np < 64 ? np : 64, q = 64 / units;
  if (NB >= q) NB -= NB % q;
  return NB;
}
__host__ __device__ inline int schur_lds_doubles(int k, int D) {
  const int WS = (D == 3) ? 18 : 26;
  return k > kSchurWideK ? k * WS + D + 1 : ((schur_nb(k) * (k * WS + D) + 1) & ~1);
}

template <int D>
__device__ __forceinline__ void schur_stage_one(bool a, const double* v, double lambda, const double* w, double* zl, double* tl, bool write_t) {
  constexpr int HU = (D == 3) ? 6 : 10;
  double L[D * (D + 1) / 2], idg[D];
  if (!a) {
#pragma unroll
    for (int i = 0; i < 6 * D; i += 2) *reinterpret_cast<double2*>(zl + i) = make_double2(0.0, 0.0);
    if (write_t) {
#pragma unroll
      for (int c = 0; c < D; c++) tl[c] = 0.0;
    }
    return;
  }
  chol_packed<D>(v, lambda, L, idg);
  double z[6 * D];
#pragma unroll
  for (int r = 0; r < 6; r++)
#pragma unroll
    for (int c = 0; c < D; c++) {
      double sacc = w[r * D + c];
#pragma unroll
      for (int m = 0; m < c; m++) sacc -= z[r * D + m] * L[c * (c + 1) / 2 + m];
      z[r * D + c] = sacc * idg[c];
    }
#pragma unroll
  for (int i = 0; i < 6 * D; i += 2) *reinterpret_cast<double2*>(zl + i) = make_double2(z[i], z[i + 1]);
  if (write_t) {
    double t[D];
#pragma unroll
    for (int c = 0; c < D; c++) {
      double sacc = v[HU + c];
#pragma unroll
      for (int m = 0; m < c; m++) sacc -= t[m] * L[c * (c + 1) / 2 + m];
      t[c] = sacc * idg[c];
    }
#pragma unroll
    for (int c = 0; c < D; c++) tl[c] = t[c];
  }
}

__device__ __forceinline__ void schur_stage_point(bool a, const double* v, double lambda, const double* G, const Vec3& Xc, double* zl, double* tl, bool write_t) {
  double L[6], idg[3];
  if (!a) {
#pragma unroll
    for (int i = 0; i < 18; i += 2) *reinterpret_cast<double2*>(zl + i) = make_double2(0.0, 0.0);
    if (write_t) { tl[0] = 0.0; tl[1] = 0.0; tl[2] = 0.0; }
    return;
  }
  chol_packed<3>(v, lambda, L, idg);
  double z[18];
#pragma unroll
  for (int r = 0; r < 3; r++)
#pragma unroll
    for (int c = 0; c < 3; c++) {
      double sacc = G[r * 3 + c];
#pragma unroll
      for (int m = 0; m < c; m++) sacc -= z[(3 + r) * 3 + m] * L[c * (c + 1) / 2 + m];
      z[(3 + r) * 3 + c] = sacc * idg[c];
    }
#pragma unroll
  for (int c = 0; c < 3; c++) {
    const double h0 = z[9 + c], h1 = z[12 + c], h2 = z[15 + c];
    z[c] = Xc.y * h2 - Xc.z * h1;
    z[3 + c] = Xc.z * h0 - Xc.x * h2;
    z[6 + c] = Xc.x * h1 - Xc.y * h0;
  }
#pragma unroll
  for (int i = 0; i < 18; i += 2) *reinterpret_cast<double2*>(zl + i) = make_double2(z[i], z[i + 1]);
  if (write_t) {
    double t[3];
#pragma unroll
    for (int c = 0; c < 3; c++) {
      double sacc = v[6 + c];
#pragma unroll
      for (int m = 0; m < c; m++) sacc -= t[m] * L[c * (c + 1) / 2 + m];
      t[c] = sacc * idg[c];
    }
    tl[0] = t[0]; tl[1] = t[1]; tl[2] = t[2];
  }
}

#ifndef LLD_SCHUR_ZFORM
#define LLD_SCHUR_HFORM 1
#endif
constexpr int kSchurHS = 14;
__device__ __forceinline__ void schur_stage_point_h(bool a, const double* v, double lambda, const double* G, const Vec3& Xc, double* zl, double* tl, bool write_t) {
  double L[6], idg[3];
  if (!a) {
#pragma unroll
    for (int i = 0; i < 12; i += 2) *reinterpret_cast<double2*>(zl + i) = make_double2(0.0, 0.0);
    if (write_t) { tl[0] = 0.0; tl[1] = 0.0; tl[2] = 0.0; }
    return;
  }
  chol_packed<3>(v, lambda, L, idg);
  double h[12];
#pragma unroll
  for (int r = 0; r < 3; r++)
#pragma unroll
    for (int c = 0; c < 3; c++) {
      double sacc = G[r * 3 + c];
#pragma unroll
      for (int m = 0; m < c; m++) sacc -= h[r * 3 + m] * L[c * (c + 1) / 2 + m];
      h[r * 3 + c] = sacc * idg[c];
    }
  h[9] = Xc.x; h[10] = Xc.y; h[11] = Xc.z;
#pragma unroll
  for (int i = 0; i < 12; i += 2) *reinterpret_cast<double2*>(zl + i) = make_double2(h[i], h[i + 1]);
  if (write_t) {
    double t[3];
#pragma unroll
    for (int c = 0; c < 3; c++) {
      double sacc = v[6 + c];
#pragma unroll
      for (int m = 0; m < c; m++) sacc -= t[m] * L[c * (c + 1) / 2 + m];
      t[c] = sacc * idg[c];
    }
    tl[0] = t[0]; tl[1] = t[1]; tl[2] = t[2];
  }
}

template <int D>
__device__ __forceinline__ void schur_chunk_wide(const BAArrays& A, const BAWin& W, const SChunk& C, double lambda, int cur, double* lds) {
  constexpr int VN = (D == 3) ? 9 : 14, WN = 6 * D, WS = (D == 3) ? 18 : 26;
  const double* __restrict__ Vbase = (D == 3) ? A.pt_V : A.ln_V;
  const uint8_t* __restrict__ act = (D == 3) ? A.pt_active : A.ln_active;
  const int k = C.k, np = k * (k + 1) / 2;
  double* Zl = lds; double* tl = lds + ((k * WS + 1) & ~1);
  for (int t0 = 0; t0 < C.n_lm; t0++) {
    const int g = A.sg_lm[C.lm_off + t0];
    const bool a = act[g] != 0;
    double v[VN];
#pragma unroll
    for (int i = 0; i < VN; i++) v[i] = Vbase[(size_t)g * VN + i];
    __syncthreads();
    for (int sl = threadIdx.x; sl < k; sl += kSchurWideThreads) {
      const int id = A.sg_tab[C.tab_off + (size_t)t0 * k + sl];
      double w[WN];
      if constexpr (D == 3) {
        const Pose Ts = load_cam(A, cur, W.cam_off + A.sg_cams[C.cams_off + sl]);
        point_hpl_closed(W.cam, Ts, quat_rotation(Ts.q), load_pt(A, cur, g), signbit(A.pe_ws[id]), fabs(A.pe_ws[id]), w);
      } else {
#pragma unroll
        for (int i = 0; i < WN; i++) w[i] = A.lo_W[(size_t)id * WN + i];
      }
      schur_stage_one<D>(a, v, lambda, w, Zl + sl * WS, tl, sl == 0);
    }
    __syncthreads();
    for (int pr = threadIdx.x; pr < np; pr += kSchurWideThreads) {
      int sa = 0, rem = pr;
      while (rem >= k - sa) { rem -= k - sa; sa++; }
      const int sb = sa + rem;
      const double* za = Zl + sa * WS; const double* zb = Zl + sb * WS;
      double* dst = A.sp_part + (size_t)(C.part_off + pr) * 36;
      for (int r = 0; r < 6; r++)
        for (int c = 0; c < 6; c++) {
          double sacc = t0 == 0 ? 0.0 : dst[r * 6 + c];
#pragma unroll
          for (int m = 0; m < D; m++) sacc = fma(za[r * D + m], zb[c * D + m], sacc);
          dst[r * 6 + c] = sacc;
        }
      if (sa == sb) {
        double* cd = A.sp_cpart + (size_t)(C.cpart_off + sa) * 6;
        for (int r = 0; r < 6; r++) {
          double sacc = t0 == 0 ? 0.0 : cd[r];
#pragma unroll
          for (int m = 0; m < D; m++) sacc = fma(za[r * D + m], tl[m], sacc);
          cd[r] = sacc;
        }
      }
    }
  }
}

template <int D>
__device__ __forceinline__ void schur_chunk_wave(const BAArrays& A, const BAWin& W, const SChunk& C, double lambda, int cur, double* lds) {
  constexpr int VN = (D == 3) ? 9 : 14, WN = 6 * D;
#ifdef LLD_SCHUR_HFORM
  constexpr bool kH = (D == 3);
  constexpr int WS = (D == 3) ? kSchurHS : 26;
#else
  constexpr bool kH = false;
  constexpr int WS = (D == 3) ? 18 : 26;
#endif
  const double* __restrict__ Vbase = (D == 3) ? A.pt_V : A.ln_V;
  const uint8_t* __restrict__ act = (D == 3) ? A.pt_active : A.ln_active;
  const int lane = threadIdx.x;
  const int k = C.k, np = k * (k + 1) / 2;
  const int NB = schur_nb(k);
  double* Zl = lds;
  double* tl = lds + NB * k * WS;
  const int* __restrict__ lm = A.sg_lm + C.lm_off;
  const int* __restrict__ tab = A.sg_tab + C.tab_off;
  const int ej = lane / k, esl = lane - ej * k;
  const bool stager = lane < NB * k;
  const int cq = (64 / k) < NB ? (64 / k) : NB;
  const int ci = lane / k, cslot = lane - ci * k;
  const bool con = ci < cq;
  double cacc[6];
#pragma unroll
  for (int i = 0; i < 6; i++) cacc[i] = 0.0;
  for (int pass0 = 0; pass0 < np; pass0 += 64) {
    const int units = (np - pass0) < 64 ? (np - pass0) : 64;
    const int q = 64 / units;
    const int pl = lane % units, qq = lane / units;
    const bool on = qq < q;
    int sa = 0, rem = pass0 + pl;
    while (rem >= k - sa) { rem -= k - sa; sa++; }
    const int sb = sa + rem;
    double acc[36];
#pragma unroll
    for (int i = 0; i < 36; i++) acc[i] = 0.0;
    Pose T; Mat3 Rt;
    if constexpr (D == 3) { if (stager) { T = load_cam(A, cur, W.cam_off + A.sg_cams[C.cams_off + esl]); Rt = quat_rotation(T.q); } }
    int g_n = 0, id_n = 0, g_nn = 0, id_nn = 0, a_n = 0;
    double v_n[VN];
    double ws_n = 0.0; Vec3 X_n = vec3(0, 0, 1);
    auto fetch_idx = [&](int t0, int& g, int& id) {
      const int tj = min(t0 + ej, C.n_lm - 1);
      g = lm[tj]; id = tab[(size_t)tj * k + esl];
    };
    auto fetch_data = [&](int t0, int g, int id) {
      a_n = act[g];
      const double* V = Vbase + (size_t)g * VN;
#pragma unroll
      for (int i = 0; i < VN; i++) v_n[i] = V[i];
      if constexpr (D == 3) { ws_n = A.pe_ws[id]; X_n = load_pt(A, cur, g); }
    };
    fetch_idx(0, g_n, id_n);
    fetch_idx(NB, g_nn, id_nn);
    fetch_data(0, g_n, id_n);
    for (int t0 = 0; t0 < C.n_lm; t0 += NB) {
      const int nb = (C.n_lm - t0) < NB ? (C.n_lm - t0) : NB;
      double w[WN], v[VN];
#pragma unroll
      for (int i = 0; i < VN; i++) v[i] = v_n[i];
      const double ws = ws_n; const Vec3 X = X_n; const int a_raw = a_n;
      const int id_cur = id_n;
      g_n = g_nn; id_n = id_nn;
      fetch_data(t0 + NB, g_n, id_n);
      fetch_idx(t0 + 2 * NB, g_nn, id_nn);
      if constexpr (D == 4) {
        const double* Wg = A.lo_W + (size_t)id_cur * WN;
#pragma unroll
        for (int i = 0; i < WN; i += 2) { const double2 t2 = *reinterpret_cast<const double2*>(Wg + i); w[i] = t2.x; w[i + 1] = t2.y; }
      }
      __syncthreads();
      if (stager && ej < nb) {
        if constexpr (D == 3) {
          const Vec3 Xc = mat_mul(Rt, X) + T.t;
          double G[9];
          point_g_closed_iz(W.cam, Xc, rcp_nr(Xc.z), Rt, signbit(ws), fabs(ws), G);
          if constexpr (kH) schur_stage_point_h(a_raw != 0, v, lambda, G, Xc, Zl + lane * WS, tl + ej * D, esl == 0);
          else schur_stage_point(a_raw != 0, v, lambda, G, Xc, Zl + lane * WS, tl + ej * D, esl == 0);
        } else schur_stage_one<D>(a_raw != 0, v, lambda, w, Zl + lane * WS, tl + ej * D, esl == 0);
      }
      __syncthreads();
      if (on) {
        for (int j = qq; j < nb; j += q) {
          const double* za = Zl + (j * k + sa) * WS;
          const double* zb = Zl + (j * k + sb) * WS;
          if constexpr (kH) {
            double ha[12], hb[12];
#pragma unroll
            for (int i = 0; i < 12; i += 2) { const double2 t2 = *reinterpret_cast<const double2*>(zb + i); hb[i] = t2.x; hb[i + 1] = t2.y; }
#pragma unroll
            for (int i = 0; i < 12; i += 2) { const double2 t2 = *reinterpret_cast<const double2*>(za + i); ha[i] = t2.x; ha[i + 1] = t2.y; }
            double M[9], P[9];
#pragma unroll
            for (int r = 0; r < 3; r++)
#pragma unroll
              for (int c = 0; c < 3; c++) M[r * 3 + c] = fma(ha[r * 3 + 2], hb[c * 3 + 2], fma(ha[r * 3 + 1], hb[c * 3 + 1], ha[r * 3] * hb[c * 3]));
            const double xa = ha[9], ya = ha[10], za_ = ha[11], xb = hb[9], yb = hb[10], zb_ = hb[11];
#pragma unroll
            for (int r = 0; r < 3; r++) {
              const double m0 = M[r * 3], m1 = M[r * 3 + 1], m2 = M[r * 3 + 2];
              P[r * 3] = fma(yb, m2, -(zb_ * m1)); P[r * 3 + 1] = fma(zb_, m0, -(xb * m2)); P[r * 3 + 2] = fma(xb, m1, -(yb * m0));
            }
#pragma unroll
            for (int c = 0; c < 3; c++) {
              acc[18 + 3 + c] += M[c]; acc[24 + 3 + c] += M[3 + c]; acc[30 + 3 + c] += M[6 + c];
              acc[18 + c] += P[c]; acc[24 + c] += P[3 + c]; acc[30 + c] += P[6 + c];
              acc[3 + c] = fma(ya, M[6 + c], fma(-za_, M[3 + c], acc[3 + c]));
              acc[6 + 3 + c] = fma(za_, M[c], fma(-xa, M[6 + c], acc[6 + 3 + c]));
              acc[12 + 3 + c] = fma(xa, M[3 + c], fma(-ya, M[c], acc[12 + 3 + c]));
              acc[c] = fma(ya, P[6 + c], fma(-za_, P[3 + c], acc[c]));
              acc[6 + c] = fma(za_, P[c], fma(-xa, P[6 + c], acc[6 + c]));
              acc[12 + c] = fma(xa, P[3 + c], fma(-ya, P[c], acc[12 + c]));
            }
            continue;
          }
          double b[WN];
#pragma unroll
          for (int i = 0; i < WN; i += 2) { const double2 t2 = *reinterpret_cast<const double2*>(zb + i); b[i] = t2.x; b[i + 1] = t2.y; }
#pragma unroll
          for (int rp = 0; rp < 3; rp++) {
            double a2[2 * D];
#pragma unroll
            for (int i = 0; i < 2 * D; i += 2) { const double2 t2 = *reinterpret_cast<const double2*>(za + rp * 2 * D + i); a2[i] = t2.x; a2[i + 1] = t2.y; }
#pragma unroll
            for (int rr = 0; rr < 2; rr++) {
              const int r = 2 * rp + rr;
#pragma unroll
              for (int cc = 0; cc < 6; cc++) {
                double s0 = acc[r * 6 + cc];
#pragma unroll
                for (int m = 0; m < D; m++) s0 = fma(a2[rr * D + m], b[cc * D + m], s0);
                acc[r * 6 + cc] = s0;
              }
            }
          }
        }
      }
      if (pass0 == 0 && con) {
        for (int j = ci; j < nb; j += cq) {
          const double* za = Zl + (j * k + cslot) * WS;
          if constexpr (kH) {
            double ha[12];
#pragma unroll
            for (int i = 0; i < 12; i += 2) { const double2 t2 = *reinterpret_cast<const double2*>(za + i); ha[i] = t2.x; ha[i + 1] = t2.y; }
            const double t0_ = tl[j * 3], t1_ = tl[j * 3 + 1], t2_ = tl[j * 3 + 2];
            const double h0 = fma(ha[2], t2_, fma(ha[1], t1_, ha[0] * t0_)), h1 = fma(ha[5], t2_, fma(ha[4], t1_, ha[3] * t0_)), h2 = fma(ha[8], t2_, fma(ha[7], t1_, ha[6] * t0_));
            cacc[3] += h0; cacc[4] += h1; cacc[5] += h2;
            cacc[0] = fma(ha[10], h2, fma(-ha[11], h1, cacc[0]));
            cacc[1] = fma(ha[11], h0, fma(-ha[9], h2, cacc[1]));
            cacc[2] = fma(ha[9], h1, fma(-ha[10], h0, cacc[2]));
            continue;
          }
          double a[WN], tv[D];
#pragma unroll
          for (int i = 0; i < WN; i += 2) { const double2 t2 = *reinterpret_cast<const double2*>(za + i); a[i] = t2.x; a[i + 1] = t2.y; }
#pragma unroll
          for (int m = 0; m < D; m++) tv[m] = tl[j * D + m];
#pragma unroll
          for (int r = 0; r < 6; r++) {
            double s1 = cacc[r];
#pragma unroll
            for (int m = 0; m < D; m++) s1 = fma(a[r * D + m], tv[m], s1);
            cacc[r] = s1;
          }
        }
      }
    }
    for (int sft = 1; sft < q; sft <<= 1) {
      const bool take = (qq % (2 * sft)) == 0 && qq + sft < q;
#pragma unroll
      for (int i = 0; i < 36; i++) { const double o = __shfl_down(acc[i], sft * units); if (take) acc[i] += o; }
    }
    if (on && qq == 0) {
      double* dst = A.sp_part + (size_t)(C.part_off + pass0 + pl) * 36;
#pragma unroll
      for (int i = 0; i < 36; i += 2) *reinterpret_cast<double2*>(dst + i) = make_double2(acc[i], acc[i + 1]);
    }
  }
  for (int sft = 1; sft < cq; sft <<= 1) {
    const bool take = (ci % (2 * sft)) == 0 && ci + sft < cq;
#pragma unroll
    for (int i = 0; i < 6; i++) { const double o = __shfl_down(cacc[i], sft * k); if (take) cacc[i] += o; }
  }
  if (ci == 0) {
    double* cd = A.sp_cpart + (size_t)(C.cpart_off + cslot) * 6;
#pragma unroll
    for (int i = 0; i < 6; i += 2) *reinterpret_cast<double2*>(cd + i) = make_double2(cacc[i], cacc[i + 1]);
  }
}

template <int D>
__global__ __launch_bounds__(kSchurThreads) void ba_schur_items_kernel(BAArrays A, const BAWin* __restrict__ wins, const BAState* __restrict__ st) {
  extern __shared__ __attribute__((aligned(16))) double lds[];
  const int wrow = LLD_ROW_WINDOW(A, st, blockIdx.y);
  if (wrow < 0) return;
  const BAWin W = wins[wrow];
  const BAState& S = st[wrow];
  if (S.phase != PH_RUN) return;
  const int first = (D == 3) ? W.item_off : W.item_off + W.n_items_pt;
  const int count = (D == 3) ? W.n_items_pt : W.n_items - W.n_items_pt;
  if ((int)blockIdx.x >= count) return;
  const SChunk C = A.sg_chunks[first + blockIdx.x];
  if (C.k <= kSchurWideK) schur_chunk_wave<D>(A, W, C, S.lambda, S.cur, lds);
}

__global__ __launch_bounds__(kSchurThreads) void ba_schur_items_both_kernel(BAArrays A, const BAWin* __restrict__ wins, const BAState* __restrict__ st, int n_pt_blocks, int win_tile, int nrow, int nch) {
  extern __shared__ __attribute__((aligned(16))) double lds[];
  const int lin = (int)blockIdx.x;
  const int tile = lin / (win_tile * nch), row0 = tile * win_tile, tsz = min(win_tile, nrow - row0), rem = lin - tile * win_tile * nch;
  const int ci = rem / tsz, row = row0 + rem - ci * tsz;
  const int wrow = LLD_ROW_WINDOW(A, st, row);
  if (wrow < 0) return;
  const BAWin W = wins[wrow];
  const BAState& S = st[wrow];
  if (S.phase != PH_RUN) return;
  if (ci < n_pt_blocks) {
    if (ci >= W.n_items_pt) return;
    const SChunk C = A.sg_chunks[W.item_off + ci];
    if (C.k <= kSchurWideK) schur_chunk_wave<3>(A, W, C, S.lambda, S.cur, lds);
  } else {
    const int i = ci - n_pt_blocks;
    if (i >= W.n_items - W.n_items_pt) return;
    const SChunk C = A.sg_chunks[W.item_off + W.n_items_pt + i];
    if (C.k <= kSchurWideK) schur_chunk_wave<4>(A, W, C, S.lambda, S.cur, lds);
  }
}

__global__ __launch_bounds__(kSchurWideThreads) void ba_schur_wide_kernel(BAArrays A, const BAWin* __restrict__ wins, const BAState* __restrict__ st) {
  extern __shared__ __attribute__((aligned(16))) double lds[];
  const int wrow = LLD_ROW_WINDOW(A, st, blockIdx.y);
  if (wrow < 0) return;
  const BAWin W = wins[wrow];
  const BAState& S = st[wrow];
  if (S.phase != PH_RUN || (int)blockIdx.x >= W.n_items) return;
  const SChunk C = A.sg_chunks[W.item_off + blockIdx.x];
  if (C.k <= kSchurWideK) return;
  if (C.D == 3) schur_chunk_wide<3>(A, W, C, S.lambda, S.cur, lds);
  else schur_chunk_wide<4>(A, W, C, S.lambda, S.cur, lds);
}

__global__ __launch_bounds__(256) __attribute__((amdgpu_waves_per_eu(5, 5))) void ba_schur_reduce_kernel(BAArrays A, const BAWin* __restrict__ wins, const BAState* __restrict__ st) {
  const int wrow = LLD_ROW_WINDOW(A, st, blockIdx.y);
  if (wrow < 0) return;
  const BAWin W = wins[wrow];
  const BAState& S = st[wrow];
  if (S.phase != PH_RUN) return;
  const int nf = W.n_free, n = 6 * nf, nblk = nf * (nf + 1) / 2;
  const int rhs_part = (int)gridDim.x - 1 - (int)blockIdx.x;
  const bool rhs_block = rhs_part < 2;
// ... 108 lines not shown
```

### lld_slam_amd/csrc/lld_device_math.h

```cpp
#ifndef LLD_DEVICE_MATH_H
#define LLD_DEVICE_MATH_H

#include <hip/hip_runtime.h>

#define LLD_HD __host__ __device__ __forceinline__

namespace lld {

struct Vec3 { double x, y, z; };
struct Mat3 { double m[3][3]; };
struct Quat { double x, y, z, w; };
struct Pose { Quat q; Vec3 t; };
struct LineQ { Quat q; double alpha; };

LLD_HD Vec3 vec3(double x, double y, double z) { Vec3 v; v.x = x; v.y = y; v.z = z; return v; }
LLD_HD Vec3 operator+(const Vec3& a, const Vec3& b) { return vec3(a.x + b.x, a.y + b.y, a.z + b.z); }
LLD_HD Vec3 operator-(const Vec3& a, const Vec3& b) { return vec3(a.x - b.x, a.y - b.y, a.z - b.z); }
LLD_HD Vec3 operator*(double s, const Vec3& a) { return vec3(s * a.x, s * a.y, s * a.z); }
LLD_HD double dot(const Vec3& a, const Vec3& b) { return a.x * b.x + a.y * b.y + a.z * b.z; }
LLD_HD Vec3 cross(const Vec3& a, const Vec3& b) {
  return vec3(a.y * b.z - a.z * b.y, a.z * b.x - a.x * b.z, a.x * b.y - a.y * b.x);
}

LLD_HD Quat quat_from_rotation(const Mat3& R) {
// ... 110 lines not shown
  return p;
}
LLD_HD void pose_store(const Pose& p, double* qt) {
  qt[0] = p.q.x; qt[1] = p.q.y; qt[2] = p.q.z; qt[3] = p.q.w; qt[4] = p.t.x; qt[5] = p.t.y; qt[6] = p.t.z;
}
LLD_HD Vec3 pose_map(const Pose& p, const Vec3& X) { return quat_rotate(p.q, X) + p.t; }

LLD_HD Pose pose_oplus(const Pose& T, const double* u) {
  const Vec3 w = vec3(u[0], u[1], u[2]), v = vec3(u[3], u[4], u[5]);
  const double theta = sqrt(dot(w, w));
  double a, b, c;
  double bv;
  if (theta < 0.00001) { a = 1.0; b = 1.0; bv = 1.0; c = 1.0; }
  else {
    const double s = sin(theta), co = cos(theta);
    a = s / theta; b = (1 - co) / (theta * theta); bv = b; c = (theta - s) / (theta * theta * theta);
  }
  const double ww = dot(w, w);
  Mat3 R;
  const double W2[3][3] = {{w.x * w.x - ww, w.x * w.y, w.x * w.z}, {w.y * w.x, w.y * w.y - ww, w.y * w.z}, {w.z * w.x, w.z * w.y, w.z * w.z - ww}};
  const double W1[3][3] = {{0, -w.z, w.y}, {w.z, 0, -w.x}, {-w.y, w.x, 0}};
#pragma unroll
  for (int i = 0; i < 3; i++) {
#pragma unroll
    for (int j = 0; j < 3; j++) R.m[i][j] = ((i == j ? 1.0 : 0.0) + a * W1[i][j]) + b * W2[i][j];
  }
  const Vec3 wv = cross(w, v);
  const Vec3 wwv = cross(w, wv);
  Pose E;
  E.q = quat_from_rotation(R);
  E.t = v + bv * wv + c * wwv;
  pose_normalize(E);
  Pose r;
  r.t = E.t + quat_rotate(E.q, T.t);
  r.q = quat_mul(E.q, T.q);
  pose_normalize(r);
  return r;
}

LLD_HD LineQ line_from_x0_dir(const Vec3& X0, const Vec3& d) {
  const double n = sqrt(dot(X0, X0));
  const Vec3 c1 = vec3(X0.x / n, X0.y / n, X0.z / n);
  const Vec3 cr = cross(d, X0);
  const Vec3 c2 = vec3(cr.x / n, cr.y / n, cr.z / n);
  Mat3 R;
  R.m[0][0] = d.x; R.m[1][0] = d.y; R.m[2][0] = d.z;
  R.m[0][1] = c1.x; R.m[1][1] = c1.y; R.m[2][1] = c1.z;
  R.m[0][2] = c2.x; R.m[1][2] = c2.y; R.m[2][2] = c2.z;
  LineQ l; l.q = quat_from_rotation(R); l.alpha = n;
  return l;
}
LLD_HD Mat3 line_rotation(const LineQ& l) { return quat_rotation(quat_unit(l.q)); }
template <bool kFast> LLD_HD Mat3 line_rotation_t(const LineQ& l) { return quat_rotation(quat_unit_t<kFast>(l.q)); }
LLD_HD LineQ line_oplus(const LineQ& l, const double* u) {
  Quat qr; qr.x = u[0]; qr.y = u[1]; qr.z = u[2];
  qr.w = sqrt(1.0 - (u[0] * u[0] + u[1] * u[1] + u[2] * u[2]));
  LineQ r; r.q = quat_mul(qr, quat_unit(l.q)); r.alpha = l.alpha + u[3];
  return r;
}

struct CamK { double fx, fy, cx, cy, bf; float bf_f; double bx_right; };
LLD_HD CamK make_camk(const lld_camera& c) {
  CamK k; k.fx = c.fx; k.fy = c.fy; k.cx = c.cx; k.cy = c.cy; k.bf = c.bf; k.bf_f = (float)c.bf;
  k.bx_right = -(double)((float)c.bf / (float)c.fx);
  return k;
}

LLD_HD void point_residual_iz(const CamK& k, const Vec3& Xc, double iz, double u, double v, double ur, bool stereo, bool binary, double* e) {
  if (stereo) {
    const float invz = (float)iz;
    const double r0 = Xc.x * (double)invz * k.fx + k.cx;
    const double r1 = Xc.y * (double)invz * k.fy + k.cy;
    const double shift = binary ? (double)(k.bf_f * invz) : k.bf * (double)invz;
    e[0] = u - r0; e[1] = v - r1; e[2] = ur - (r0 - shift);
  } else {
    e[0] = u - (Xc.x * iz * k.fx + k.cx);
    e[1] = v - (Xc.y * iz * k.fy + k.cy);
    e[2] = 0.0;
  }
}
LLD_HD void point_residual(const CamK& k, const Vec3& Xc, double u, double v, double ur, bool stereo, bool binary, double* e) {
  if (stereo) {
    const float invz = (float)(1.0 / Xc.z);
    const double r0 = Xc.x * (double)invz * k.fx + k.cx;
    const double r1 = Xc.y * (double)invz * k.fy + k.cy;
    const double shift = binary ? (double)(k.bf_f * invz) : k.bf * (double)invz;
    e[0] = u - r0; e[1] = v - r1; e[2] = ur - (r0 - shift);
  } else {
    e[0] = u - (Xc.x / Xc.z * k.fx + k.cx);
    e[1] = v - (Xc.y / Xc.z * k.fy + k.cy);
    e[2] = 0.0;
  }
}

LLD_HD void point_jac_pose(const CamK& k, const Vec3& Xc, bool stereo, double* Jc) {
  const double x = Xc.x, y = Xc.y, iz = 1.0 / Xc.z, iz2 = iz * iz;
  Jc[0] = x * y * iz2 * k.fx;
  Jc[1] = -(1 + x * x * iz2) * k.fx;
  Jc[2] = y * iz * k.fx;
  Jc[3] = -iz * k.fx;
  Jc[4] = 0;
  Jc[5] = x * iz2 * k.fx;
  Jc[6] = (1 + y * y * iz2) * k.fy;
  Jc[7] = -x * y * iz2 * k.fy;
  Jc[8] = -x * iz * k.fy;
  Jc[9] = 0;
  Jc[10] = -iz * k.fy;
  Jc[11] = y * iz2 * k.fy;
  if (stereo) {
    Jc[12] = Jc[0] - k.bf * y * iz2;
    Jc[13] = Jc[1] + k.bf * x * iz2;
    Jc[14] = Jc[2];
    Jc[15] = Jc[3];
    Jc[16] = 0;
    Jc[17] = Jc[5] - k.bf * iz2;
  } else {
    Jc[12] = Jc[13] = Jc[14] = Jc[15] = Jc[16] = Jc[17] = 0;
  }
}
LLD_HD void point_jac_point(const CamK& k, const Vec3& Xc, const Mat3& R, bool stereo, double* Jp) {
  const double iz = 1.0 / Xc.z, iz2 = iz * iz;
  for (int j = 0; j < 3; j++) {
    Jp[j] = -k.fx * R.m[0][j] * iz + k.fx * Xc.x * R.m[2][j] * iz2;
    Jp[3 + j] = -k.fy * R.m[1][j] * iz + k.fy * Xc.y * R.m[2][j] * iz2;
    Jp[6 + j] = stereo ? Jp[j] - k.bf * R.m[2][j] * iz2 : 0.0;
  }
}

LLD_HD void point_hpl_closed_iz(const CamK& k, const Vec3& Xc, double iz, const Mat3& R, bool stereo, double ws, double* W);
LLD_HD void point_hpl_closed(const CamK& k, const Pose& T, const Mat3& R, const Vec3& X, bool stereo, double ws, double* W) {
  const Vec3 Xc = mat_mul(R, X) + T.t;
  point_hpl_closed_iz(k, Xc, 1.0 / Xc.z, R, stereo, ws, W);
}
LLD_HD void point_hpl_closed_iz(const CamK& k, const Vec3& Xc, double iz, const Mat3& R, bool stereo, double ws, double* W) {
  const double iz2 = iz * iz;
  const double a = k.fx * iz, b = k.fy * iz;
  const double c0 = -k.fx * Xc.x * iz2, c1 = -k.fy * Xc.y * iz2, c2 = c0 + k.bf * iz2;
  const double m00 = ws * (stereo ? 2.0 * a * a : a * a);
  const double m02 = ws * (stereo ? a * (c0 + c2) : a * c0);
  const double m11 = ws * (b * b), m12 = ws * (b * c1);
  const double m22 = ws * (stereo ? c0 * c0 + c1 * c1 + c2 * c2 : c0 * c0 + c1 * c1);
#pragma unroll
  for (int j = 0; j < 3; j++) {
    const double g0 = m00 * R.m[0][j] + m02 * R.m[2][j];
    const double g1 = m11 * R.m[1][j] + m12 * R.m[2][j];
    const double g2 = m02 * R.m[0][j] + m12 * R.m[1][j] + m22 * R.m[2][j];
    W[0 * 3 + j] = Xc.y * g2 - Xc.z * g1;
    W[1 * 3 + j] = Xc.z * g0 - Xc.x * g2;
    W[2 * 3 + j] = Xc.x * g1 - Xc.y * g0;
    W[3 * 3 + j] = g0; W[4 * 3 + j] = g1; W[5 * 3 + j] = g2;
  }
}

LLD_HD void point_g_closed_iz(const CamK& k, const Vec3& Xc, double iz, const Mat3& R, bool stereo, double ws, double* G) {
  const double iz2 = iz * iz;
  const double a = k.fx * iz, b = k.fy * iz;
  const double c0 = -k.fx * Xc.x * iz2, c1 = -k.fy * Xc.y * iz2, c2 = c0 + k.bf * iz2;
  const double m00 = ws * (stereo ? 2.0 * a * a : a * a);
  const double m02 = ws * (stereo ? a * (c0 + c2) : a * c0);
  const double m11 = ws * (b * b), m12 = ws * (b * c1);
  const double m22 = ws * (stereo ? c0 * c0 + c1 * c1 + c2 * c2 : c0 * c0 + c1 * c1);
#pragma unroll
  for (int j = 0; j < 3; j++) {
    G[j] = m00 * R.m[0][j] + m02 * R.m[2][j];
    G[3 + j] = m11 * R.m[1][j] + m12 * R.m[2][j];
    G[6 + j] = m02 * R.m[0][j] + m12 * R.m[1][j] + m22 * R.m[2][j];
  }
}

struct LineAdj { Vec3 a1[2], a2[2]; };
template <bool kFast>
LLD_HD void line_residual_t(const CamK& k, double bx, const Vec3& X1m, const Vec3& X2m, double xs, double ys, double xe, double ye,
                            double* e, LineAdj* adj) {
  const double f = k.fx;
  const Vec3 P1 = vec3(f * (X1m.x + bx) + k.cx * X1m.z, f * X1m.y + k.cy * X1m.z, X1m.z);
  const Vec3 P2 = vec3(f * (X2m.x + bx) + k.cx * X2m.z, f * X2m.y + k.cy * X2m.z, X2m.z);
  const Vec3 lt = cross(P1, P2);
  const double n2 = lt.x * lt.x + lt.y * lt.y;
  double in;
  if (kFast) in = rsqrt_nr(n2); else { const double n = sqrt(n2); in = 1.0 / n; }
  const double d1 = xs * lt.x + ys * lt.y + lt.z, d2 = xe * lt.x + ye * lt.y + lt.z;
  e[0] = d1 * in; e[1] = d2 * in;
  if (adj) {
    const double in3 = kFast ? in * in * in : in / n2;
    const double px[2] = {xs, xe}, py[2] = {ys, ye}, dd[2] = {d1, d2};
    for (int q = 0; q < 2; q++) {
      const Vec3 g = vec3(px[q] * in - dd[q] * in3 * lt.x, py[q] * in - dd[q] * in3 * lt.y, in);
      const Vec3 h1 = cross(P2, g), h2 = cross(g, P1);
      adj->a1[q] = vec3(f * h1.x, f * h1.y, k.cx * h1.x + k.cy * h1.y + h1.z);
      adj->a2[q] = vec3(f * h2.x, f * h2.y, k.cx * h2.x + k.cy * h2.y + h2.z);
    }
  }
}
LLD_HD void line_residual(const CamK& k, double bx, const Vec3& X1m, const Vec3& X2m, double xs, double ys, double xe, double ye,
                          double* e, LineAdj* adj) { line_residual_t<false>(k, bx, X1m, X2m, xs, ys, xe, ye, e, adj); }
LLD_HD void line_jac_pose(const LineAdj& adj, const Vec3& X1m, const Vec3& X2m, double* Jc) {
  for (int q = 0; q < 2; q++) {
    const Vec3 r = cross(X1m, adj.a1[q]) + cross(X2m, adj.a2[q]);
    const Vec3 s = adj.a1[q] + adj.a2[q];
    Jc[q * 6 + 0] = r.x; Jc[q * 6 + 1] = r.y; Jc[q * 6 + 2] = r.z;
    Jc[q * 6 + 3] = s.x; Jc[q * 6 + 4] = s.y; Jc[q * 6 + 5] = s.z;
  }
}
LLD_HD void line_jac_line(const LineAdj& adj, const Mat3& Rcam, const Vec3& c0, const Vec3& c1, double alpha, double* Jl) {
  const Vec3 X1 = alpha * c1;
  for (int q = 0; q < 2; q++) {
    const Vec3 b1 = mat_tmul(Rcam, adj.a1[q]), b2 = mat_tmul(Rcam, adj.a2[q]);
    const Vec3 bs = b1 + b2;
    const Vec3 r = 2.0 * (cross(X1, bs) + cross(c0, b2));
    Jl[q * 4 + 0] = r.x; Jl[q * 4 + 1] = r.y; Jl[q * 4 + 2] = r.z; Jl[q * 4 + 3] = dot(bs, c1);
  }
}

LLD_HD double reproject_depth(const CamK& k, const Vec3& X0, const Vec3& ld, double px, double py) {
  const double f = k.fx;
  const Vec3 a = vec3(px, py, 1.0);
  const Vec3 b = vec3(-(f * ld.x + k.cx * ld.z), -(f * ld.y + k.cy * ld.z), -ld.z);
  const Vec3 r = vec3(f * X0.x + k.cx * X0.z, f * X0.y + k.cy * X0.z, X0.z);
  const double aa = dot(a, a), ab = dot(a, b), bb = dot(b, b), ar = dot(a, r), br = dot(b, r);
  return (bb * ar - ab * br) / (aa * bb - ab * ab);
}
LLD_HD bool line_depth_positive(const CamK& k, double bx, const Pose& T, const Vec3& c0, const Vec3& c1, double alpha,
                                double xs, double ys, double xe, double ye) {
  const Vec3 X0 = alpha * c1;
  Vec3 X0l = pose_map(T, X0); X0l.x += bx;
  Vec3 X1l = pose_map(T, X0 + c0); X1l.x += bx;
  const Vec3 ldl = X1l - X0l;
  const double d1 = reproject_depth(k, X0l, ldl, xs, ys);
  const double d2 = reproject_depth(k, X0l, ldl, xe, ye);
  return !(d1 < 0 || d2 < 0);
}

LLD_HD double huber_nr(double e, double delta, double* rho1) {
  const double dsqr = delta * delta;
  const bool in = e <= dsqr;
  const double is = rsqrt_nr(in ? 1.0 : e);
  *rho1 = in ? 1.0 : delta * is;
  return in ? e : 2 * (e * is) * delta - dsqr;
}
LLD_HD double huber(double e, double delta, double* rho1) {
  const double dsqr = delta * delta;
  if (e <= dsqr) { *rho1 = 1.0; return e; }
  const double s = sqrt(e);
  *rho1 = delta / s;
  return 2 * s * delta - dsqr;
}

LLD_HD double line_info(double gamma, int octave) {
  double t = 1.0;
  for (int i = 0; i < octave; i++) t *= 1.44;
  double info = 1.0 * (gamma * gamma);
  info /= t * t;
  return info;
}

}
#endif
```

Before: 6163.

## Fold point-edge camera Hessian blocks into Schur diagonal update

Point linearization no longer accumulates the full 21-entry camera Hpp block per point edge. It keeps only the gradient (6 values) and, on the first iteration, the Hpp diagonal (6 values) for the LM lambda init. The point-edge camera self-term is instead added during the Schur complement. Staging now carries the per-edge M matrix entries so diagonal pairs subtract it, and a separate hdiag buffer supplies the lambda-init max. This cuts atomics and LDS traffic in linearization and shrinks hpart storage, at the cost of extra Schur arithmetic, larger staging records (14 to 18 doubles), and some code paths recomputing M per edge.

```diff
diff --git a/lld_slam_amd/csrc/lld_ba.hip b/lld_slam_amd/csrc/lld_ba.hip
--- a/lld_slam_amd/csrc/lld_ba.hip
+++ b/lld_slam_amd/csrc/lld_ba.hip
@@ -607,18 +607,21 @@
   if (P.deterministic < 0 || P.deterministic > 2) return fail(LLD_ERR_INVALID);
   if (B->big && P.deterministic == 1) return fail(LLD_ERR_UNSUPPORTED);
   const bool det = P.deterministic != 0 && !B->big;
-  auto lin_lds_bytes = [&](int copies) { return ((size_t)B->max_free * 27 * copies + 8 + (size_t)B->max_cams * 7) * sizeof(double); };
-  int copies = B->big ? 1 : kAccCopies;
-  while (!B->big && copies > 1 && lin_lds_bytes(copies) > 150 * 1024) copies >>= 1;
-  if (!B->big && lin_lds_bytes(copies) > 158 * 1024) return fail(LLD_ERR_UNSUPPORTED);
-  B->acc_copies[0] = B->acc_copies[1] = copies;
-  B->lin_waves[0] = det ? copies : kLinThreads / 64;
-  B->lin_waves[1] = det ? copies : (n_windows >= 64 ? 4 : kLinThreads / 64);
+  auto lin_lds_bytes = [&](int copies, int per_cam) { return ((size_t)B->max_free * per_cam * copies + 8 + (size_t)B->max_cams * 7) * sizeof(double); };
+  for (int kind = 0; kind < 2; kind++) {
+    const int per_cam = kind == 0 ? (int)hpart_pt_row(1, true) : 27;
+    int copies = B->big ? 1 : kAccCopies;
+    while (!B->big && copies > 1 && lin_lds_bytes(copies, per_cam) > 150 * 1024) copies >>= 1;
+    if (!B->big && lin_lds_bytes(copies, per_cam) > 158 * 1024) return fail(LLD_ERR_UNSUPPORTED);
+    B->acc_copies[kind] = copies;
+  }
+  B->lin_waves[0] = det ? B->acc_copies[0] : kLinThreads / 64;
+  B->lin_waves[1] = det ? B->acc_copies[1] : (n_windows >= 64 ? 4 : kLinThreads / 64);
   if (const char* e = exp_str("LLD_BA_LIN_WAVES")) {
     int a = 0, c = 0;
     if (std::sscanf(e, "%d,%d", &a, &c) == 2 && a >= 1 && a <= 8 && c >= 1 && c <= 8) {
       B->lin_waves[0] = a; B->lin_waves[1] = c;
-      if (det) { B->acc_copies[0] = a; B->acc_copies[1] = c; if (lin_lds_bytes(std::max(a, c)) > 158 * 1024) return fail(LLD_ERR_UNSUPPORTED); }
+      if (det) { B->acc_copies[0] = a; B->acc_copies[1] = c; if (lin_lds_bytes(a, 12) > 158 * 1024 || lin_lds_bytes(c, 27) > 158 * 1024) return fail(LLD_ERR_UNSUPPORTED); }
     }
   }
   std::vector<WinStage> stages(n_windows);
@@ -726,7 +729,8 @@
       W.ptask_off = (int)q.ptask; W.ltask_off = (int)q.ltask; W.item_off = (int)q.chunk;
       W.n_items_pt = (int)S.cs[0].chunks.size(); W.n_items = W.n_items_pt + (int)S.cs[1].chunks.size();
       W.blk_csr_off = (int)q.blk_start; W.cam_csr_off = (int)q.cam_start;
-      W.hpart_off = (long long)n_hpart; n_hpart += (size_t)(big_map ? 1 : W.nl_pt + W.nl_ln) * W.n_free * 27;
+      W.hpart_off = (long long)n_hpart;
+      n_hpart += big_map ? (size_t)W.n_free * 27 : (size_t)W.nl_pt * hpart_pt_row(W.n_free, true) + (size_t)W.nl_ln * W.n_free * 27;
       W.part_off = (int)NPART; NPART += W.nt_pt + W.nt_ln;
       q.ptask += S.ptasks.size(); q.ltask += S.ltasks.size(); q.chunk += (size_t)W.n_items;
       q.lm += S.cs[0].sg_lm.size() + S.cs[1].sg_lm.size(); q.tab += S.cs[0].sg_tab.size() + S.cs[1].sg_tab.size(); q.cams += S.cs[0].sg_cams.size() + S.cs[1].sg_cams.size();
@@ -751,7 +755,7 @@
   const bool s_skip_empty = (P.reduced_solver == 0 || P.reduced_solver >= 3) && B->max_free * 6 <= kCholMN && !B->pcg_multi;
   if (B->max_free > kMaxFreeCamsOneWg && !B->pcg_multi) return fail(LLD_ERR_UNSUPPORTED);
   if (B->max_cams > kPcgThreads && !B->pcg_multi) return fail(LLD_ERR_UNSUPPORTED);
-  for (int wi = 0; wi < n_windows; wi++) { B->h_wins[wi].acc_copies[0] = B->acc_copies[0]; B->h_wins[wi].acc_copies[1] = B->acc_copies[1]; B->h_wins[wi].win_index = wi; B->h_wins[wi].big = B->big ? 1 : 0; }
+  for (int wi = 0; wi < n_windows; wi++) { B->h_wins[wi].acc_copies[0] = B->acc_copies[0]; B->h_wins[wi].acc_copies[1] = B->acc_copies[1]; B->h_wins[wi].win_index = wi; B->h_wins[wi].big = B->big ? 1 : 0; B->h_wins[wi].fold = B->big ? 0 : 1; }
   B->max_blk = max_blk;
   for (int wi = 0; wi < n_windows; wi++) B->h_wins[wi].rec_off = (long long)(B->rec_stride * (size_t)wi);
   const size_t rec_total = B->rec_stride * (size_t)n_windows;
@@ -784,7 +788,7 @@
     A.pt_active = sl.take<uint8_t>(NP + 1); A.ln_active = sl.take<uint8_t>(NL + 1); A.ln_removed = sl.take<uint8_t>(NL + 1);
     A.pt_V = sl.take<double>((size_t)NP * 9 + 1); A.ln_V = sl.take<double>((size_t)NL * 14 + 1);
     A.hpp_part = sl.take<double>(n_hpart + 2);
-    A.Hpp = sl.take<double>((size_t)NF * 21 + 1); A.bp = sl.take<double>((size_t)NF * 6 + 1);
+    A.Hpp = sl.take<double>((size_t)NF * 21 + 1); A.bp = sl.take<double>((size_t)NF * 6 + 1); A.hdiag = sl.take<double>((size_t)NF * 6 + 1);
     A.S = sl.take<double>(S_total + 1); A.bschur = sl.take<double>(x_total + 1); A.xp = sl.take<double>(x_total + 1);
     A.x_total = (long long)x_total; A.s_skip_empty = s_skip_empty ? 1 : 0;
     if (B->pcg_multi) { A.pcg_vec = sl.take<double>(4 * x_total + 4); A.pcg_mi = sl.take<double>((size_t)NF * 36 + 1); A.pcg_sc = sl.take<double>(8 * (size_t)n_windows + 8); }
@@ -929,7 +933,7 @@
   for (auto& l : B->launches) l = 0;
   B->super_steps = 0;
   LLD_HIP_TRY(hipEventRecord(t_begin, ctx->stream));
-  const size_t lin_lds_pt = B->big ? 64 : ((size_t)B->max_free * 27 * B->acc_copies[0] + 8 + (size_t)B->max_cams * 7) * sizeof(double);
+  const size_t lin_lds_pt = B->big ? 64 : ((size_t)hpart_pt_row(B->max_free, true) * B->acc_copies[0] + 8 + (size_t)B->max_cams * 7) * sizeof(double);
   const size_t lin_lds_ln = B->big ? 64 : ((size_t)B->max_free * 27 * B->acc_copies[1] + 8 + (size_t)B->max_cams * 7) * sizeof(double);
   const bool same_lin_shape = B->lin_waves[0] == B->lin_waves[1] && B->acc_copies[0] == B->acc_copies[1];
   const size_t bs_lds = B->big ? 64 : (8 + (size_t)B->max_cams * 14 + (size_t)B->max_free * 6) * sizeof(double);
@@ -973,7 +977,7 @@
     if (B->big) {
       if (G.max_nl_pt > 0) hipLaunchKernelGGL(ba_linearize_pt_big_kernel, dim3(G.max_nl_pt, nw), dim3(64 * B->lin_waves[0]), lin_lds_pt, st, A, dw, ds);
       if (G.max_nl_ln > 0) hipLaunchKernelGGL(ba_linearize_ln_big_kernel, dim3(G.max_nl_ln, nw), dim3(64 * B->lin_waves[1]), lin_lds_ln, st, A, dw, ds);
-    } else if (fuse_pairs && same_lin_shape && G.max_nl_pt > 0 && G.max_nl_ln > 0) hipLaunchKernelGGL(ba_linearize_both_kernel, dim3(G.max_nl_pt + G.max_nl_ln, nw), dim3(64 * B->lin_waves[0]), lin_lds_pt, st, A, dw, ds, G.max_nl_pt);
+    } else if (fuse_pairs && same_lin_shape && G.max_nl_pt > 0 && G.max_nl_ln > 0) hipLaunchKernelGGL(ba_linearize_both_kernel, dim3(G.max_nl_pt + G.max_nl_ln, nw), dim3(64 * B->lin_waves[0]), std::max(lin_lds_pt, lin_lds_ln), st, A, dw, ds, G.max_nl_pt);
     else {
       if (G.max_nl_pt > 0) hipLaunchKernelGGL(packed ? ba_linearize_pt_kernel : ba_linearize_pt_f64_kernel, dim3(G.max_nl_pt, nw), dim3(64 * B->lin_waves[0]), lin_lds_pt, st, A, dw, ds);
       if (G.max_nl_ln > 0) hipLaunchKernelGGL(packed ? ba_linearize_ln_kernel : ba_linearize_ln_f64_kernel, dim3(G.max_nl_ln, nw), dim3(64 * B->lin_waves[1]), lin_lds_ln, st, A, dw, ds);
diff --git a/lld_slam_amd/csrc/lld_ba_kernels.h b/lld_slam_amd/csrc/lld_ba_kernels.h
--- a/lld_slam_amd/csrc/lld_ba_kernels.h
+++ b/lld_slam_amd/csrc/lld_ba_kernels.h
@@ -22,6 +22,7 @@
 constexpr int kRoundsBigMinWindows = 192;
 constexpr int kAccCopies = 4;
 constexpr int kAccCopiesDoc = 4;
+__host__ __device__ inline long long hpart_pt_row(int n_free, bool fold) { return (long long)n_free * (fold ? 12 : 27); }
 constexpr int kMaxFreeCams = 8192;
 constexpr int kMaxFreeCamsLds = 590;
 constexpr int kMaxFreeCamsOneWg = 170;
@@ -55,6 +56,7 @@
   int max_trials, ln_filter;
   int abort_after;
   int big;
+  int fold;
   int protocol, robust_pts;
   int acc_copies[2];
   int det, lin_waves[2];
@@ -113,6 +115,7 @@
   double *ln_V;
   double *hpp_part;
   double *Hpp;
+  double *hdiag;
   double *bp;
   double *S, *bschur, *xp;
   double *pcg_vec;
diff --git a/lld_slam_amd/csrc/lld_ba_lines.h b/lld_slam_amd/csrc/lld_ba_lines.h
--- a/lld_slam_amd/csrc/lld_ba_lines.h
+++ b/lld_slam_amd/csrc/lld_ba_lines.h
@@ -174,7 +174,7 @@
   }
   __syncthreads();
   if (kBig) return;
-  double* dst = A.hpp_part + W.hpart_off + (size_t)(W.nl_pt + bx) * nacc;
+  double* dst = A.hpp_part + W.hpart_off + (size_t)W.nl_pt * hpart_pt_row(W.n_free, W.fold) + (size_t)bx * nacc;
   for (int i = threadIdx.x; i < nacc; i += nthr) {
     double v = 0.0;
     for (int q = 0; q < copies; q++) v += acc_all[q * nacc + i];
@@ -333,11 +333,8 @@
   chi = wave_sum(chi);
   double md = 0.0;
   if (S.it == 0) {
-    const double* H = A.Hpp + (size_t)W.hpp_off * 21;
-    for (int c = lane; c < W.n_free; c += 64) {
-      const double* h = H + c * 21;
-      md = fmax(md, fmax(fmax(fabs(xwg_load(h)), fabs(xwg_load(h + 6))), fmax(fmax(fabs(xwg_load(h + 11)), fabs(xwg_load(h + 15))), fmax(fabs(xwg_load(h + 18)), fabs(xwg_load(h + 20))))));
-    }
+    const double* H = A.hdiag + (size_t)W.hpp_off * 6;
+    for (int i = lane; i < W.n_free * 6; i += 64) md = fmax(md, fabs(xwg_load(H + i)));
     md = wave_max(md);
   }
   if (lane == 0) {
@@ -348,6 +345,20 @@
     }
     S.q = 0; S.need_lin = 0;
   }
+}
+
+__device__ __forceinline__ double hpart_sum(const double* src, int nb, size_t stride) {
+  double v = 0.0;
+  int b = 0;
+  for (; b + 8 <= nb; b += 8) {
+    double t[8];
+#pragma unroll
+    for (int u = 0; u < 8; u++) t[u] = src[(size_t)(b + u) * stride];
+#pragma unroll
+    for (int u = 0; u < 8; u++) v += t[u];
+  }
+  for (; b < nb; b++) v += src[(size_t)b * stride];
+  return v;
 }
 
 __global__ __launch_bounds__(256) void ba_hpp_reduce_kernel(BAArrays A, const BAWin* __restrict__ wins, BAState* __restrict__ st) {
@@ -360,20 +371,19 @@
   const int nacc = W.n_free * 27;
   const int i = blockIdx.x * 256 + threadIdx.x;
   if (i < nacc) {
-    const double* src = A.hpp_part + W.hpart_off + i;
-    const int nb = W.big ? 1 : W.nl_pt + W.nl_ln;
-    double v = 0.0;
-    int b = 0;
-    for (; b + 8 <= nb; b += 8) {
-      double t[8];
-#pragma unroll
-      for (int u = 0; u < 8; u++) t[u] = src[(size_t)(b + u) * nacc];
-#pragma unroll
-      for (int u = 0; u < 8; u++) v += t[u];
-    }
-    for (; b < nb; b++) v += src[(size_t)b * nacc];
     const int c = i / 27, k = i - c * 27;
+    const double* part = A.hpp_part + W.hpart_off;
+    const size_t prow = (size_t)hpart_pt_row(W.n_free, W.fold);
+    double v, vd = 0.0;
+    const int r = k == 0 ? 0 : k == 6 ? 1 : k == 11 ? 2 : k == 15 ? 3 : k == 18 ? 4 : k == 20 ? 5 : -1;
+    if (!W.fold) v = hpart_sum(part + i, W.big ? 1 : W.nl_pt + W.nl_ln, nacc);
+    else {
+      v = hpart_sum(part + W.nl_pt * prow + i, W.nl_ln, nacc);
+      if (k >= 21) v += hpart_sum(part + c * 6 + (k - 21), W.nl_pt, prow);
+      else if (r >= 0 && S.it == 0) vd = hpart_sum(part + (size_t)W.n_free * 6 + c * 6 + r, W.nl_pt, prow);
+    }
     if (k < 21) xwg_store(&A.Hpp[((size_t)W.hpp_off + c) * 21 + k], v); else A.bp[((size_t)W.hpp_off + c) * 6 + (k - 21)] = v;
+    if (r >= 0 && S.it == 0) xwg_store(&A.hdiag[((size_t)W.hpp_off + c) * 6 + r], v + vd);
   }
   xwg_stores_done();
   __syncthreads();
diff --git a/lld_slam_amd/csrc/lld_ba_points.h b/lld_slam_amd/csrc/lld_ba_points.h
--- a/lld_slam_amd/csrc/lld_ba_points.h
+++ b/lld_slam_amd/csrc/lld_ba_points.h
@@ -81,7 +81,16 @@
     for (int cc = rr; cc < 6; cc++) atomicAdd(&ac[kk++], L.ws * (L.Jc[rr] * L.Jc[cc] + L.Jc[6 + rr] * L.Jc[6 + cc] + L.Jc[12 + rr] * L.Jc[12 + cc]));
   }
 }
-
+__device__ __forceinline__ void point_edge_bp(const PtEdgeLin& L, double* bp, double* dg) {
+#pragma unroll
+  for (int rr = 0; rr < 6; rr++) atomicAdd(&bp[rr], -L.ws * (L.Jc[rr] * L.r[0] + L.Jc[6 + rr] * L.r[1] + L.Jc[12 + rr] * L.r[2]));
+  if (dg) {
+#pragma unroll
+    for (int rr = 0; rr < 6; rr++) atomicAdd(&dg[rr], L.ws * (L.Jc[rr] * L.Jc[rr] + L.Jc[6 + rr] * L.Jc[6 + rr] + L.Jc[12 + rr] * L.Jc[12 + rr]));
+  }
+}
+
+template <bool kFold>
 __device__ __forceinline__ double point_edge_blocks_closed(const BAWin& W, const Pose& T, const Vec3& X, const PtObs& ob, uint8_t fl, double& ws_out,
                                                            double& rho0_out, double* hb, double* hp) {
   const CamK& k = W.cam;
@@ -119,6 +128,14 @@
 #pragma unroll
   for (int p = 0; p < 3; p++) hb[6 + p] = R.m[0][p] * g0 + R.m[1][p] * g1 + R.m[2][p] * g2;
   const double x = Xc.x, y = Xc.y, z = Xc.z;
+  if constexpr (kFold) {
+    hp[0] = y * g2 - z * g1; hp[1] = z * g0 - x * g2; hp[2] = x * g1 - y * g0; hp[3] = g0; hp[4] = g1; hp[5] = g2;
+    const double p01 = y * m12 - z * m11, p02 = y * m22 - z * m12, p10 = z * m00 - x * m02, p12 = z * m02 - x * m22;
+    const double p20 = -(y * m00), p21 = x * m11;
+    hp[6] = y * p02 - z * p01; hp[7] = z * p10 - x * p12; hp[8] = x * p21 - y * p20;
+    hp[9] = m00; hp[10] = m11; hp[11] = m22;
+    return c2e;
+  }
   const double P[3][3] = {{y * m02 - z * 0.0, y * m12 - z * m11, y * m22 - z * m12},
                           {z * m00 - x * m02, z * 0.0 - x * m12, z * m02 - x * m22},
                           {x * 0.0 - y * m00, x * m11 - y * 0.0, x * m12 - y * m02}};
@@ -142,11 +159,13 @@
   BAState& S = st[wrow];
   if (S.phase != PH_RUN || !S.need_lin) return;
   if ((int)bx >= W.nl_pt) return;
-  const int nacc = W.n_free * 27;
+  constexpr bool kFold = !kBig;
+  const bool dg = S.it == 0;
+  const int nacc = kFold ? W.n_free * (dg ? 12 : 6) : W.n_free * 27;
   const int cur = S.cur;
   double* acc_all = kBig ? A.hpp_part + W.hpart_off : lds;
   const int copies = W.acc_copies[0];
-  double* scratch = kBig ? lds : lds + copies * nacc;
+  double* scratch = kBig ? lds : lds + copies * W.n_free * 12;
   double* cams_l = scratch + 8;
   const double* cams = kBig ? A.cam_qt + ((size_t)cur * A.NC + W.cam_off) * 7 : cams_l;
   double* acc = acc_all;
@@ -187,14 +206,25 @@
       for (int i = 0; i < 9; i++) hb[i] = 0.0;
       if (has && (fl & EF_LEVEL1)) A.pe_ws[e] = 0.0;
       if (lm_act && !(fl & EF_LEVEL1)) {
-        double hp[27], ws_e, rho0_e;
-        A.pe_chi2[e] = point_edge_blocks_closed(W, pose_load(cams + c * 7), X, ob, fl, ws_e, rho0_e, hb, hp);
+        double hp[kFold ? 12 : 27], ws_e, rho0_e;
+        A.pe_chi2[e] = point_edge_blocks_closed<kFold>(W, pose_load(cams + c * 7), X, ob, fl, ws_e, rho0_e, hb, hp);
         A.pe_ws[e] = (fl & EF_STEREO) ? -ws_e : ws_e;
         chi += rho0_e;
         if (c < W.n_free) {
-          double* ac = acc + c * 27;
-#pragma unroll
-          for (int i = 0; i < 27; i++) if (i != 16) atomicAdd(&ac[i], hp[i]);
+          if constexpr (kFold) {
+            double* ac = acc + c * 6;
+#pragma unroll
+            for (int i = 0; i < 6; i++) atomicAdd(&ac[i], hp[i]);
+            if (dg) {
+              double* ad = acc + W.n_free * 6 + c * 6;
+#pragma unroll
+              for (int i = 0; i < 6; i++) atomicAdd(&ad[i], hp[6 + i]);
+            }
+          } else {
+            double* ac = acc + c * 27;
+#pragma unroll
+            for (int i = 0; i < 27; i++) if (i != 16) atomicAdd(&ac[i], hp[i]);
+          }
         }
       }
       seg_sum<9>(hb, l, lane, T.ms);
@@ -223,7 +253,10 @@
           point_edge_hll(L, h1);
 #pragma unroll
           for (int i = 0; i < 9; i++) hb[i] += h1[i];
-          if (c < W.n_free) point_edge_hpp(L, acc + c * 27);
+          if (c < W.n_free) {
+            if constexpr (kFold) point_edge_bp(L, acc + c * 6, dg ? acc + W.n_free * 6 + c * 6 : nullptr);
+            else point_edge_hpp(L, acc + c * 27);
+          }
         }
         wave_sum_n<9>(hb);
         if (lane == 0) {
@@ -243,7 +276,7 @@
   }
   __syncthreads();
   if (kBig) return;
-  double* dst = A.hpp_part + W.hpart_off + (size_t)(bx) * nacc;
+  double* dst = A.hpp_part + W.hpart_off + (size_t)bx * hpart_pt_row(W.n_free, true);
   for (int i = threadIdx.x; i < nacc; i += nthr) {
     double v = 0.0;
     for (int q = 0; q < copies; q++) v += acc_all[q * nacc + i];
diff --git a/lld_slam_amd/csrc/lld_ba_schur.h b/lld_slam_amd/csrc/lld_ba_schur.h
--- a/lld_slam_amd/csrc/lld_ba_schur.h
+++ b/lld_slam_amd/csrc/lld_ba_schur.h
@@ -52,73 +52,32 @@
   }
 }
 
-__device__ __forceinline__ void schur_stage_point(bool a, const double* v, double lambda, const double* G, const Vec3& Xc, double* zl, double* tl, bool write_t) {
+constexpr int kSchurHS = 18;
+__device__ __forceinline__ void schur_stage_point_h(bool a, const double* v, double lambda, const double* G, const Vec3& Xc, const double* me, double* zl, double* tl, bool write_t) {
   double L[6], idg[3];
   if (!a) {
 #pragma unroll
-    for (int i = 0; i < 18; i += 2) *reinterpret_cast<double2*>(zl + i) = make_double2(0.0, 0.0);
+    for (int i = 0; i < kSchurHS; i += 2) *reinterpret_cast<double2*>(zl + i) = make_double2(0.0, 0.0);
     if (write_t) { tl[0] = 0.0; tl[1] = 0.0; tl[2] = 0.0; }
     return;
   }
   chol_packed<3>(v, lambda, L, idg);
-  double z[18];
+  double h[kSchurHS];
 #pragma unroll
   for (int r = 0; r < 3; r++)
 #pragma unroll
     for (int c = 0; c < 3; c++) {
       double sacc = G[r * 3 + c];
 #pragma unroll
-      for (int m = 0; m < c; m++) sacc -= z[(3 + r) * 3 + m] * L[c * (c + 1) / 2 + m];
-      z[(3 + r) * 3 + c] = sacc * idg[c];
-    }
-#pragma unroll
-  for (int c = 0; c < 3; c++) {
-    const double h0 = z[9 + c], h1 = z[12 + c], h2 = z[15 + c];
-    z[c] = Xc.y * h2 - Xc.z * h1;
-    z[3 + c] = Xc.z * h0 - Xc.x * h2;
-    z[6 + c] = Xc.x * h1 - Xc.y * h0;
-  }
-#pragma unroll
-  for (int i = 0; i < 18; i += 2) *reinterpret_cast<double2*>(zl + i) = make_double2(z[i], z[i + 1]);
-  if (write_t) {
-    double t[3];
-#pragma unroll
-    for (int c = 0; c < 3; c++) {
-      double sacc = v[6 + c];
-#pragma unroll
-      for (int m = 0; m < c; m++) sacc -= t[m] * L[c * (c + 1) / 2 + m];
-      t[c] = sacc * idg[c];
-    }
-    tl[0] = t[0]; tl[1] = t[1]; tl[2] = t[2];
-  }
-}
-
-#ifndef LLD_SCHUR_ZFORM
-#define LLD_SCHUR_HFORM 1
-#endif
-constexpr int kSchurHS = 14;
-__device__ __forceinline__ void schur_stage_point_h(bool a, const double* v, double lambda, const double* G, const Vec3& Xc, double* zl, double* tl, bool write_t) {
-  double L[6], idg[3];
-  if (!a) {
-#pragma unroll
-    for (int i = 0; i < 12; i += 2) *reinterpret_cast<double2*>(zl + i) = make_double2(0.0, 0.0);
-    if (write_t) { tl[0] = 0.0; tl[1] = 0.0; tl[2] = 0.0; }
-    return;
-  }
-  chol_packed<3>(v, lambda, L, idg);
-  double h[12];
-#pragma unroll
-  for (int r = 0; r < 3; r++)
-#pragma unroll
-    for (int c = 0; c < 3; c++) {
-      double sacc = G[r * 3 + c];
-#pragma unroll
       for (int m = 0; m < c; m++) sacc -= h[r * 3 + m] * L[c * (c + 1) / 2 + m];
       h[r * 3 + c] = sacc * idg[c];
     }
   h[9] = Xc.x; h[10] = Xc.y; h[11] = Xc.z;
 #pragma unroll
-  for (int i = 0; i < 12; i += 2) *reinterpret_cast<double2*>(zl + i) = make_double2(h[i], h[i + 1]);
+  for (int i = 0; i < 5; i++) h[12 + i] = me[i];
+  h[17] = 0.0;
+#pragma unroll
+  for (int i = 0; i < kSchurHS; i += 2) *reinterpret_cast<double2*>(zl + i) = make_double2(h[i], h[i + 1]);
   if (write_t) {
     double t[3];
 #pragma unroll
@@ -172,6 +131,22 @@
           for (int m = 0; m < D; m++) sacc = fma(za[r * D + m], zb[c * D + m], sacc);
           dst[r * 6 + c] = sacc;
         }
+      if constexpr (D == 3) {
+        if (sa == sb && W.fold && a) {
+          const int id = A.sg_tab[C.tab_off + (size_t)t0 * k + sa];
+          const Pose Ts = load_cam(A, cur, W.cam_off + A.sg_cams[C.cams_off + sa]);
+          const Vec3 Xc = mat_mul(quat_rotation(Ts.q), load_pt(A, cur, g)) + Ts.t;
+          double me[5];
+          point_m_closed_iz(W.cam, Xc, 1.0 / Xc.z, signbit(A.pe_ws[id]), fabs(A.pe_ws[id]), me);
+          const double M[3][3] = {{me[0], 0.0, me[1]}, {0.0, me[2], me[3]}, {me[1], me[3], me[4]}};
+          const double Bm[6][3] = {{0.0, -Xc.z, Xc.y}, {Xc.z, 0.0, -Xc.x}, {-Xc.y, Xc.x, 0.0}, {1.0, 0.0, 0.0}, {0.0, 1.0, 0.0}, {0.0, 0.0, 1.0}};
+          for (int r = 0; r < 6; r++) {
+            double bm[3];
+            for (int m = 0; m < 3; m++) bm[m] = Bm[r][0] * M[0][m] + Bm[r][1] * M[1][m] + Bm[r][2] * M[2][m];
+            for (int c = 0; c < 6; c++) dst[r * 6 + c] -= bm[0] * Bm[c][0] + bm[1] * Bm[c][1] + bm[2] * Bm[c][2];
+          }
+        }
+      }
       if (sa == sb) {
         double* cd = A.sp_cpart + (size_t)(C.cpart_off + sa) * 6;
         for (int r = 0; r < 6; r++) {
@@ -188,13 +163,8 @@
 template <int D>
 __device__ __forceinline__ void schur_chunk_wave(const BAArrays& A, const BAWin& W, const SChunk& C, double lambda, int cur, double* lds) {
   constexpr int VN = (D == 3) ? 9 : 14, WN = 6 * D;
-#ifdef LLD_SCHUR_HFORM
   constexpr bool kH = (D == 3);
   constexpr int WS = (D == 3) ? kSchurHS : 26;
-#else
-  constexpr bool kH = false;
-  constexpr int WS = (D == 3) ? 18 : 26;
-#endif
   const double* __restrict__ Vbase = (D == 3) ? A.pt_V : A.ln_V;
   const uint8_t* __restrict__ act = (D == 3) ? A.pt_active : A.ln_active;
   const int lane = threadIdx.x;
@@ -220,6 +190,7 @@
     int sa = 0, rem = pass0 + pl;
     while (rem >= k - sa) { rem -= k - sa; sa++; }
     const int sb = sa + rem;
+    const double dgm = sa == sb ? -1.0 : 0.0;
     double acc[36];
 #pragma unroll
     for (int i = 0; i < 36; i++) acc[i] = 0.0;
@@ -261,10 +232,13 @@
       if (stager && ej < nb) {
         if constexpr (D == 3) {
           const Vec3 Xc = mat_mul(Rt, X) + T.t;
-          double G[9];
-          point_g_closed_iz(W.cam, Xc, rcp_nr(Xc.z), Rt, signbit(ws), fabs(ws), G);
-          if constexpr (kH) schur_stage_point_h(a_raw != 0, v, lambda, G, Xc, Zl + lane * WS, tl + ej * D, esl == 0);
-          else schur_stage_point(a_raw != 0, v, lambda, G, Xc, Zl + lane * WS, tl + ej * D, esl == 0);
+          double G[9], me[5];
+          point_g_closed_iz(W.cam, Xc, rcp_nr(Xc.z), Rt, signbit(ws), fabs(ws), G, me);
+          if (!W.fold) {
+#pragma unroll
+            for (int i = 0; i < 5; i++) me[i] = 0.0;
+          }
+          schur_stage_point_h(a_raw != 0, v, lambda, G, Xc, me, Zl + lane * WS, tl + ej * D, esl == 0);
         } else schur_stage_one<D>(a_raw != 0, v, lambda, w, Zl + lane * WS, tl + ej * D, esl == 0);
       }
       __syncthreads();
@@ -278,11 +252,16 @@
             for (int i = 0; i < 12; i += 2) { const double2 t2 = *reinterpret_cast<const double2*>(zb + i); hb[i] = t2.x; hb[i + 1] = t2.y; }
 #pragma unroll
             for (int i = 0; i < 12; i += 2) { const double2 t2 = *reinterpret_cast<const double2*>(za + i); ha[i] = t2.x; ha[i + 1] = t2.y; }
+            const double2 e01 = *reinterpret_cast<const double2*>(za + 12), e23 = *reinterpret_cast<const double2*>(za + 14);
+            const double e4 = za[16];
             double M[9], P[9];
 #pragma unroll
             for (int r = 0; r < 3; r++)
 #pragma unroll
               for (int c = 0; c < 3; c++) M[r * 3 + c] = fma(ha[r * 3 + 2], hb[c * 3 + 2], fma(ha[r * 3 + 1], hb[c * 3 + 1], ha[r * 3] * hb[c * 3]));
+            M[0] = fma(dgm, e01.x, M[0]); M[2] = fma(dgm, e01.y, M[2]); M[6] = fma(dgm, e01.y, M[6]);
+            M[4] = fma(dgm, e23.x, M[4]); M[5] = fma(dgm, e23.y, M[5]); M[7] = fma(dgm, e23.y, M[7]);
+            M[8] = fma(dgm, e4, M[8]);
             const double xa = ha[9], ya = ha[10], za_ = ha[11], xb = hb[9], yb = hb[10], zb_ = hb[11];
 #pragma unroll
             for (int r = 0; r < 3; r++) {
diff --git a/lld_slam_amd/csrc/lld_device_math.h b/lld_slam_amd/csrc/lld_device_math.h
--- a/lld_slam_amd/csrc/lld_device_math.h
+++ b/lld_slam_amd/csrc/lld_device_math.h
@@ -286,14 +286,18 @@
   }
 }
 
-LLD_HD void point_g_closed_iz(const CamK& k, const Vec3& Xc, double iz, const Mat3& R, bool stereo, double ws, double* G) {
+LLD_HD void point_m_closed_iz(const CamK& k, const Vec3& Xc, double iz, bool stereo, double ws, double* m) {
   const double iz2 = iz * iz;
   const double a = k.fx * iz, b = k.fy * iz;
   const double c0 = -k.fx * Xc.x * iz2, c1 = -k.fy * Xc.y * iz2, c2 = c0 + k.bf * iz2;
-  const double m00 = ws * (stereo ? 2.0 * a * a : a * a);
-  const double m02 = ws * (stereo ? a * (c0 + c2) : a * c0);
-  const double m11 = ws * (b * b), m12 = ws * (b * c1);
-  const double m22 = ws * (stereo ? c0 * c0 + c1 * c1 + c2 * c2 : c0 * c0 + c1 * c1);
+  m[0] = ws * (stereo ? 2.0 * a * a : a * a);
+  m[1] = ws * (stereo ? a * (c0 + c2) : a * c0);
+  m[2] = ws * (b * b); m[3] = ws * (b * c1);
+  m[4] = ws * (stereo ? c0 * c0 + c1 * c1 + c2 * c2 : c0 * c0 + c1 * c1);
+}
+LLD_HD void point_g_closed_iz(const CamK& k, const Vec3& Xc, double iz, const Mat3& R, bool stereo, double ws, double* G, double* m) {
+  point_m_closed_iz(k, Xc, iz, stereo, ws, m);
+  const double m00 = m[0], m02 = m[1], m11 = m[2], m12 = m[3], m22 = m[4];
 #pragma unroll
   for (int j = 0; j < 3; j++) {
     G[j] = m00 * R.m[0][j] + m02 * R.m[2][j];
```

After: 6309 (median of 6 runs). +2.4%, better.
